# foges/pogs

Hardware: AMD Instinct MI355X
Metric: admm_iterations_per_sec_dense_lasso_fp32 (per-GPU shard, summed over GPUs) (higher is better)
Workload: dtype f32

## Files before the change

include/pogs_amd.h:

```cpp
#ifndef POGS_AMD_H_
#define POGS_AMD_H_

#include <stddef.h>

#ifdef __cplusplus
extern "C" {
#endif


enum ORD { COL_MAJ, ROW_MAJ };

enum FUNCTION { ABS, EXP, HUBER, IDENTITY, INDBOX01, INDEQ0, INDGE0, INDLE0,
                LOGISTIC, MAXNEG0, MAXPOS0, NEGENTR, NEGLOG, RECIPR, SQUARE, ZERO };

enum POGS_STATUS { POGS_SUCCESS = 0, POGS_INFEASIBLE = 1, POGS_UNBOUNDED = 2,
                   POGS_MAX_ITER = 3, POGS_NAN_FOUND = 4, POGS_INVALID_CONE = 5,
                   POGS_ERROR = 6 };

int PogsD(enum ORD ord, size_t m, size_t n, const double *A,
          const double *f_a, const double *f_b, const double *f_c,
          const double *f_d, const double *f_e, const enum FUNCTION *f_h,
          const double *g_a, const double *g_b, const double *g_c,
          const double *g_d, const double *g_e, const enum FUNCTION *g_h,
          double rho, double abs_tol, double rel_tol, unsigned int max_iter,
          unsigned int verbose, int adaptive_rho, int gap_stop,
          double *x, double *y, double *l, double *optval, unsigned int *final_iter);

int PogsS(enum ORD ord, size_t m, size_t n, const float *A,
          const float *f_a, const float *f_b, const float *f_c,
          const float *f_d, const float *f_e, const enum FUNCTION *f_h,
          const float *g_a, const float *g_b, const float *g_c,
          const float *g_d, const float *g_e, const enum FUNCTION *g_h,
          float rho, float abs_tol, float rel_tol, unsigned int max_iter,
          unsigned int verbose, int adaptive_rho, int gap_stop,
          float *x, float *y, float *l, float *optval, unsigned int *final_iter);

int PogsSparseD(enum ORD ord, size_t m, size_t n, size_t nnz,
                const double *data, const int *ptr, const int *ind,
                const double *f_a, const double *f_b, const double *f_c,
                const double *f_d, const double *f_e, const enum FUNCTION *f_h,
                const double *g_a, const double *g_b, const double *g_c,
                const double *g_d, const double *g_e, const enum FUNCTION *g_h,
                double rho, double abs_tol, double rel_tol, unsigned int max_iter,
                unsigned int verbose, int adaptive_rho, int gap_stop,
                double *x, double *y, double *l, double *optval,
                unsigned int *final_iter);

int PogsSparseS(enum ORD ord, size_t m, size_t n, size_t nnz,
                const float *data, const int *ptr, const int *ind,
                const float *f_a, const float *f_b, const float *f_c,
                const float *f_d, const float *f_e, const enum FUNCTION *f_h,
                const float *g_a, const float *g_b, const float *g_c,
                const float *g_d, const float *g_e, const enum FUNCTION *g_h,
                float rho, float abs_tol, float rel_tol, unsigned int max_iter,
                unsigned int verbose, int adaptive_rho, int gap_stop,
                float *x, float *y, float *l, float *optval,
                unsigned int *final_iter);


typedef struct PogsAmdSolver PogsAmdSolver;

enum POGS_AMD_DTYPE { POGS_AMD_F32 = 0, POGS_AMD_F64 = 1 };
enum POGS_AMD_MEM { POGS_AMD_HOST = 0, POGS_AMD_DEVICE = 1 };
enum POGS_AMD_PROJECTOR { POGS_AMD_PROJ_DEFAULT = 0,
                          POGS_AMD_PROJ_DIRECT = 1, POGS_AMD_PROJ_CGLS = 2 };

#define POGS_AMD_UNIQUE_ID_BYTES 128

typedef struct PogsAmdDist {
  int rank;
  int world;
  size_t m_global;
  char unique_id[POGS_AMD_UNIQUE_ID_BYTES];
} PogsAmdDist;

typedef struct PogsAmdOptions {
  int device;
  int projector;
  int profile;
  int reserved[5];
} PogsAmdOptions;

typedef struct PogsAmdStats {
  double t_total_s, t_init_s, t_loop_s, t_h2d_s;
  unsigned int iterations;
  unsigned int exact_iters;
  unsigned int norm_est_iters;
  unsigned int rho_updates;
  unsigned long long cg_iters;
  unsigned long long matvecs;
  unsigned long long matvecs_init;
  double rho_final, nrmA;
  double stream_ms;
  unsigned long long stream_launches;
  double stream_bytes;
  double equil_ms, normest_ms, gram_ms, chol_ms, trtri_ms;
  double gram_flops;
  double reserved[8];
} PogsAmdStats;

int PogsAmdDistUniqueId(char *out);

int PogsAmdCreateDense(PogsAmdSolver **out, int dtype, enum ORD ord, size_t m,
                       size_t n, const void *A, int mem,
                       const PogsAmdOptions *opt, const PogsAmdDist *dist);

int PogsAmdCreateSparse(PogsAmdSolver **out, int dtype, enum ORD ord, size_t m,
                        size_t n, size_t nnz, const void *data, const int *ptr,
                        const int *ind, int mem, const PogsAmdOptions *opt,
                        const PogsAmdDist *dist);

int PogsAmdSolve(PogsAmdSolver *s,
                 const void *f_a, const void *f_b, const void *f_c, const void *f_d,
                 const void *f_e, const int *f_h,
                 const void *g_a, const void *g_b, const void *g_c, const void *g_d,
                 const void *g_e, const int *g_h,
                 double rho, double abs_tol, double rel_tol, unsigned int max_iter,
                 unsigned int verbose, int adaptive_rho, int gap_stop,
                 void *x, void *y, void *l, void *mu, double *optval,
                 unsigned int *final_iter);

typedef struct PogsAmdFn {
  const void *a, *b, *c, *d, *e;
  const int *h;
  double a0, b0, c0, d0, e0;
  int h0;
} PogsAmdFn;
int PogsAmdSolveFn(PogsAmdSolver *s, const PogsAmdFn *f, const PogsAmdFn *g,
                   double rho, double abs_tol, double rel_tol, unsigned int max_iter,
                   unsigned int verbose, int adaptive_rho, int gap_stop,
                   void *x, void *y, void *l, void *mu, double *optval,
                   unsigned int *final_iter);
int PogsAmdBeginRunFn(PogsAmdSolver *s, const PogsAmdFn *f, const PogsAmdFn *g,
                      double rho, double abs_tol, double rel_tol, unsigned int max_iter,
                      int adaptive_rho, int gap_stop);

#define POGS_AMD_BATCH_MAX 16
int PogsAmdSolveBatchFn(PogsAmdSolver *s, int k, const PogsAmdFn *f, const PogsAmdFn *g, const double *rho,
                        double abs_tol, double rel_tol, unsigned int max_iter, unsigned int verbose,
                        int adaptive_rho, int gap_stop, void *x, void *y, void *l, void *mu,
                        double *optval, unsigned int *final_iter, int *status);

int PogsAmdSolveBatchSparseFn(PogsAmdSolver *s, int k, const PogsAmdFn *f, const PogsAmdFn *g, const double *rho,
                              double abs_tol, double rel_tol, unsigned int max_iter, unsigned int verbose,
                              int adaptive_rho, int gap_stop, void *x, void *y, void *l, void *mu,
                              double *optval, unsigned int *final_iter, int *status);

#define POGS_AMD_MANY_MIN_DIM_MAX 512
#define POGS_AMD_MANY_MAX_DIM_MAX 16384
int PogsAmdSolveManyFn(int dtype, enum ORD ord, int k, size_t m, size_t n, const void *A, int mem,
                       const PogsAmdOptions *opt, const PogsAmdFn *f, const PogsAmdFn *g, const double *rho,
                       double abs_tol, double rel_tol, unsigned int max_iter, unsigned int verbose,
                       int adaptive_rho, int gap_stop, void *x, void *y, void *l, void *mu,
                       double *optval, unsigned int *final_iter, int *status);

int PogsAmdBeginRun(PogsAmdSolver *s,
                    const void *f_a, const void *f_b, const void *f_c, const void *f_d,
                    const void *f_e, const int *f_h,
                    const void *g_a, const void *g_b, const void *g_c, const void *g_d,
                    const void *g_e, const int *g_h,
                    double rho, double abs_tol, double rel_tol, unsigned int max_iter,
                    int adaptive_rho, int gap_stop);
int PogsAmdIterate(PogsAmdSolver *s, unsigned int iters, double *seconds,
                   unsigned int *solves_completed);

int PogsAmdSetWarmStart(PogsAmdSolver *s, const void *x0, const void *l0);

int PogsAmdGetStats(const PogsAmdSolver *s, PogsAmdStats *out);
int PogsAmdResetStats(PogsAmdSolver *s);
void PogsAmdDestroy(PogsAmdSolver *s);

const char *PogsAmdLastError(void);

typedef struct PogsAmdPoolInfo {
  unsigned long long mallocs;
  unsigned long long reuses;
  unsigned long long frees;
  double malloc_ms, free_ms;
  size_t cached_bytes;
  size_t live_bytes;
  size_t peak_cached_bytes;
} PogsAmdPoolInfo;
int PogsAmdPoolStats(int device, PogsAmdPoolInfo *out);
int PogsAmdPoolTrim(int device, size_t *freed_bytes);


int PogsAmdProxEval(int dtype, size_t n, const int *h, const void *a, const void *b,
                    const void *c, const void *d, const void *e, double rho,
                    const void *in, void *out);
int PogsAmdFuncEval(int dtype, size_t n, const int *h, const void *a, const void *b,
                    const void *c, const void *d, const void *e, const void *in,
                    double *out);
int PogsAmdProjSubgradEval(int dtype, size_t n, const int *h, const void *a, const void *b,
                           const void *c, const void *d, const void *e, const void *x_in,
                           const void *v_in, void *v_out);
int PogsAmdGetEquil(const PogsAmdSolver *s, void *A_eq, void *d, void *e, double *nrmA);
int PogsAmdProject(PogsAmdSolver *s, const void *x0, const void *y0, double tol,
                   void *x, void *y);
int PogsAmdMul(PogsAmdSolver *s, char trans, double alpha, const void *x, double beta,
               void *y);
int PogsAmdReadBandwidth(int device, size_t bytes, int reps, double *gb_per_s, int *pattern);
int PogsAmdWaveSumCheck(int dtype, size_t n, const void *in_host, void *alu_host, void *lds_host);

int PogsAmdBatchRowsCheck(int dtype, int tri, int rows, int cols, const void *M, size_t ldm, int k, const int *act,
                          int nact, const void *X, size_t ldx, void *Y, size_t ldy);
int PogsAmdBatchColsCheck(int dtype, int rows, int cols, const void *M, size_t ldm, int k, const int *act, int nact,
                          const void *U, size_t ldu, const void *add, void *Z, size_t ldz, int *nrb_used, int *rpb);
int PogsAmdSpBatchSpmvCheck(int dtype, int nrows, int ncols, const int *ptr, const int *ind, const void *val, int k,
                            const int *act, int nact, const void *X, size_t ldx, double beta, const void *yin,
                            size_t ldin, void *Y, size_t ldy, double *part, int num_cu, int *geom);
int PogsAmdManySetupCheck(int dtype, enum ORD ord, int k, size_t m, size_t n, const void *A, int mem, void *A_eq,
                          void *d, void *e, double *nrmA, void *W);
int PogsAmdGramCheck(int dtype, int kdim, int k, const void *P, size_t lda, int num_cu, int force, void *G, size_t ldg,
                     int *info);
int PogsAmdCholCheck(int dtype, int n, const void *H, size_t ldh, void *L, void *W, void *U, size_t ldo);
int PogsAmdSpmvCheck(int dtype, enum ORD ord, int nrows, int ncols, const int *ptr, const int *ind, const void *val,
                     int num_cu, int format, int force_rr_rows, int force_ncg, double scale, char trans, int sq,
                     double x_nrm2, double alpha, double beta, const void *x, size_t xlen, void *y, size_t ylen,
                     double *sumsq, int *info, int *t_ptr, int *t_ind, void *t_val);
int PogsAmdGetFactor(const PogsAmdSolver *s, void *W, void *U);
int PogsAmdRandUniform(int dtype, size_t n, void *out_host);

#ifdef __cplusplus
}
#endif
#endif
```

pogs_amd/_lib.py:

```python
import ctypes
import os
import sys

_PKG = os.path.dirname(os.path.abspath(__file__))
LIB_PATH = os.path.join(_PKG, "libpogs_amd.so")

TORCH_LOADED_FIRST = "torch" in sys.modules
if not TORCH_LOADED_FIRST and os.environ.get("POGS_AMD_TORCH_PRELOAD", "0") == "1":
    try:
        import torch

        TORCH_LOADED_FIRST = True
    except ImportError:
        pass


def check_device_pointer_interop():
    if "torch" in sys.modules and not TORCH_LOADED_FIRST:
        raise RuntimeError(
            "pogs_amd was imported before torch: the two then run on separate HIP runtimes and a torch device "
            "pointer is not valid here.  Import torch first, or set POGS_AMD_TORCH_PRELOAD=1.")


if not os.path.exists(LIB_PATH):
    raise ImportError(
        "pogs_amd: %s not found. Build it with:\n"
        "  python pogs_amd/build.py        (needs hipcc; cross-compiles for gfx950 without a GPU)\n" % LIB_PATH
    )

lib = ctypes.CDLL(LIB_PATH)

c_int, c_uint, c_size_t, c_double, c_float, c_void_p, c_char = (
    ctypes.c_int, ctypes.c_uint, ctypes.c_size_t, ctypes.c_double, ctypes.c_float, ctypes.c_void_p, ctypes.c_char)

UNIQUE_ID_BYTES = 128
F32, F64 = 0, 1
HOST, DEVICE = 0, 1
COL_MAJ, ROW_MAJ = 0, 1
PROJ_DEFAULT, PROJ_DIRECT, PROJ_CGLS = 0, 1, 2


class PogsAmdDist(ctypes.Structure):
    _fields_ = [("rank", c_int), ("world", c_int), ("m_global", c_size_t), ("unique_id", c_char * UNIQUE_ID_BYTES)]


class PogsAmdOptions(ctypes.Structure):
    _fields_ = [("device", c_int), ("projector", c_int), ("profile", c_int), ("reserved", c_int * 5)]


class PogsAmdStats(ctypes.Structure):
    _fields_ = [
        ("t_total_s", c_double), ("t_init_s", c_double), ("t_loop_s", c_double), ("t_h2d_s", c_double),
        ("iterations", c_uint), ("exact_iters", c_uint), ("norm_est_iters", c_uint), ("rho_updates", c_uint),
        ("cg_iters", ctypes.c_ulonglong), ("matvecs", ctypes.c_ulonglong), ("matvecs_init", ctypes.c_ulonglong),
        ("rho_final", c_double), ("nrmA", c_double),
        ("stream_ms", c_double), ("stream_launches", ctypes.c_ulonglong), ("stream_bytes", c_double),
        ("equil_ms", c_double), ("normest_ms", c_double), ("gram_ms", c_double), ("chol_ms", c_double),
        ("trtri_ms", c_double), ("gram_flops", c_double), ("reserved", c_double * 8),
    ]

    def as_dict(self):
        d = {k: getattr(self, k) for k, _ in self._fields_ if k != "reserved"}
        d["spec_hits"], d["spec_misses"] = self.reserved[0], self.reserved[1]
        d["collectives"] = int(self.reserved[2])
        d["comm_nranks"] = int(self.reserved[3])
        d["batch_problem_iters"] = int(self.reserved[4])
        d["batch_pass_ms"], d["batch_pass_launches"] = self.reserved[5], int(self.reserved[6])
        d["batch_pass_bytes"] = self.reserved[7]
        return d


def _dense_sig(real):
    return [c_int, c_size_t, c_size_t, c_void_p] + [c_void_p] * 5 + [c_void_p] + [c_void_p] * 5 + [c_void_p] + \
        [real, real, real, c_uint, c_uint, c_int, c_int, c_void_p, c_void_p, c_void_p, c_void_p, c_void_p]


def _sparse_sig(real):
    return [c_int, c_size_t, c_size_t, c_size_t, c_void_p, c_void_p, c_void_p] + [c_void_p] * 5 + [c_void_p] + \
        [c_void_p] * 5 + [c_void_p] + [real, real, real, c_uint, c_uint, c_int, c_int,
                                        c_void_p, c_void_p, c_void_p, c_void_p, c_void_p]


lib.PogsD.argtypes = _dense_sig(c_double)
lib.PogsS.argtypes = _dense_sig(c_float)
lib.PogsSparseD.argtypes = _sparse_sig(c_double)
lib.PogsSparseS.argtypes = _sparse_sig(c_float)
for _f in (lib.PogsD, lib.PogsS, lib.PogsSparseD, lib.PogsSparseS):
    _f.restype = c_int

lib.PogsAmdDistUniqueId.argtypes = [c_void_p]
lib.PogsAmdCreateDense.argtypes = [ctypes.POINTER(c_void_p), c_int, c_int, c_size_t, c_size_t, c_void_p, c_int,
                                   ctypes.POINTER(PogsAmdOptions), ctypes.POINTER(PogsAmdDist)]
lib.PogsAmdCreateSparse.argtypes = [ctypes.POINTER(c_void_p), c_int, c_int, c_size_t, c_size_t, c_size_t, c_void_p,
                                    c_void_p, c_void_p, c_int, ctypes.POINTER(PogsAmdOptions),
                                    ctypes.POINTER(PogsAmdDist)]
lib.PogsAmdSolve.argtypes = [c_void_p] + [c_void_p] * 12 + [c_double, c_double, c_double, c_uint, c_uint, c_int, c_int,
                                                            c_void_p, c_void_p, c_void_p, c_void_p,
                                                            ctypes.POINTER(c_double), ctypes.POINTER(c_uint)]
class PogsAmdFn(ctypes.Structure):
    _fields_ = [("a", c_void_p), ("b", c_void_p), ("c", c_void_p), ("d", c_void_p), ("e", c_void_p), ("h", c_void_p),
                ("a0", c_double), ("b0", c_double), ("c0", c_double), ("d0", c_double), ("e0", c_double), ("h0", c_int)]


lib.PogsAmdSolveFn.argtypes = [c_void_p, ctypes.POINTER(PogsAmdFn), ctypes.POINTER(PogsAmdFn), c_double, c_double, c_double,
                               c_uint, c_uint, c_int, c_int, c_void_p, c_void_p, c_void_p, c_void_p,
                               ctypes.POINTER(c_double), ctypes.POINTER(c_uint)]
lib.PogsAmdSolveBatchFn.argtypes = [c_void_p, c_int, ctypes.POINTER(PogsAmdFn), ctypes.POINTER(PogsAmdFn), c_void_p,
                                    c_double, c_double, c_uint, c_uint, c_int, c_int, c_void_p, c_void_p, c_void_p,
                                    c_void_p, c_void_p, c_void_p, c_void_p]
lib.PogsAmdSolveBatchSparseFn.argtypes = lib.PogsAmdSolveBatchFn.argtypes
BATCH_MAX = 16
lib.PogsAmdSolveManyFn.argtypes = [c_int, c_int, c_int, c_size_t, c_size_t, c_void_p, c_int, ctypes.POINTER(PogsAmdOptions),
                                   ctypes.POINTER(PogsAmdFn), ctypes.POINTER(PogsAmdFn), c_void_p, c_double, c_double,
                                   c_uint, c_uint, c_int, c_int, c_void_p, c_void_p, c_void_p, c_void_p, c_void_p,
                                   c_void_p, c_void_p]
MANY_MIN_DIM_MAX = 512
MANY_MAX_DIM_MAX = 16384
lib.PogsAmdBeginRunFn.argtypes = [c_void_p, ctypes.POINTER(PogsAmdFn), ctypes.POINTER(PogsAmdFn), c_double, c_double, c_double,
                                  c_uint, c_int, c_int]
lib.PogsAmdBeginRun.argtypes = [c_void_p] + [c_void_p] * 12 + [c_double, c_double, c_double, c_uint, c_int, c_int]
lib.PogsAmdIterate.argtypes = [c_void_p, c_uint, ctypes.POINTER(c_double), ctypes.POINTER(c_uint)]
lib.PogsAmdSetWarmStart.argtypes = [c_void_p, c_void_p, c_void_p]
lib.PogsAmdGetStats.argtypes = [c_void_p, ctypes.POINTER(PogsAmdStats)]
lib.PogsAmdResetStats.argtypes = [c_void_p]
lib.PogsAmdDestroy.argtypes = [c_void_p]
lib.PogsAmdDestroy.restype = None
lib.PogsAmdLastError.restype = ctypes.c_char_p
lib.PogsAmdProxEval.argtypes = [c_int, c_size_t] + [c_void_p] * 6 + [c_double, c_void_p, c_void_p]
lib.PogsAmdFuncEval.argtypes = [c_int, c_size_t] + [c_void_p] * 6 + [c_void_p, ctypes.POINTER(c_double)]
lib.PogsAmdProjSubgradEval.argtypes = [c_int, c_size_t] + [c_void_p] * 6 + [c_void_p, c_void_p, c_void_p]
lib.PogsAmdGetEquil.argtypes = [c_void_p, c_void_p, c_void_p, c_void_p, ctypes.POINTER(c_double)]
lib.PogsAmdProject.argtypes = [c_void_p, c_void_p, c_void_p, c_double, c_void_p, c_void_p]
lib.PogsAmdMul.argtypes = [c_void_p, c_char, c_double, c_void_p, c_double, c_void_p]
lib.PogsAmdRandUniform.argtypes = [c_int, c_size_t, c_void_p]
lib.PogsAmdReadBandwidth.argtypes = [c_int, c_size_t, c_int, ctypes.POINTER(c_double), ctypes.POINTER(c_int)]
lib.PogsAmdWaveSumCheck.argtypes = [c_int, c_size_t, c_void_p, c_void_p, c_void_p]
lib.PogsAmdBatchRowsCheck.argtypes = [c_int, c_int, c_int, c_int, c_void_p, c_size_t, c_int, c_void_p, c_int,
                                      c_void_p, c_size_t, c_void_p, c_size_t]
lib.PogsAmdBatchColsCheck.argtypes = [c_int, c_int, c_int, c_void_p, c_size_t, c_int, c_void_p, c_int, c_void_p,
                                      c_size_t, c_void_p, c_void_p, c_size_t, ctypes.POINTER(c_int),
                                      ctypes.POINTER(c_int)]
lib.PogsAmdSpBatchSpmvCheck.argtypes = [c_int, c_int, c_int, c_void_p, c_void_p, c_void_p, c_int, c_void_p, c_int,
                                        c_void_p, c_size_t, c_double, c_void_p, c_size_t, c_void_p, c_size_t, c_void_p,
                                        c_int, c_void_p]
lib.PogsAmdManySetupCheck.argtypes = [c_int, c_int, c_int, c_size_t, c_size_t, c_void_p, c_int, c_void_p, c_void_p,
                                      c_void_p, c_void_p, c_void_p]
lib.PogsAmdGramCheck.argtypes = [c_int, c_int, c_int, c_void_p, c_size_t, c_int, c_int, c_void_p, c_size_t, c_void_p]
lib.PogsAmdCholCheck.argtypes = [c_int, c_int, c_void_p, c_size_t, c_void_p, c_void_p, c_void_p, c_size_t]
lib.PogsAmdSpmvCheck.argtypes = [c_int, c_int, c_int, c_int, c_void_p, c_void_p, c_void_p, c_int, c_int, c_int, c_int,
                                 c_double, c_char, c_int, c_double, c_double, c_double, c_void_p, c_size_t, c_void_p,
                                 c_size_t, ctypes.POINTER(c_double), c_void_p, c_void_p, c_void_p, c_void_p]
lib.PogsAmdGetFactor.argtypes = [c_void_p, c_void_p, c_void_p]
GRAM_AUTO, GRAM_NATIVE, GRAM_TILE_128, GRAM_TILE_256 = 0, 1, 128, 256
GRAM_INFO = ("path", "tile", "ksplit", "kchunk", "kacc", "units", "unit_rows", "tile_map")
SPMV_AUTO, SPMV_TAGS, SPMV_TWO, SPMV_PLAIN = 0, 1, 2, 3
SPMV_INFO = ("tiled", "two", "rr_rows", "nrr", "ncb", "ncg", "units", "why")
SPMV_WHY = {0: "tiled", 1: "no non-zeros", 2: "plan too large", 3: "planner range", 4: "padding", 5: "row count over 16 bits",
            6: "pinned plain"}


class PogsAmdPoolInfo(ctypes.Structure):
    _fields_ = [("mallocs", ctypes.c_ulonglong), ("reuses", ctypes.c_ulonglong), ("frees", ctypes.c_ulonglong),
                ("malloc_ms", c_double), ("free_ms", c_double), ("cached_bytes", c_size_t), ("live_bytes", c_size_t),
                ("peak_cached_bytes", c_size_t)]


lib.PogsAmdPoolStats.argtypes = [c_int, ctypes.POINTER(PogsAmdPoolInfo)]
lib.PogsAmdPoolTrim.argtypes = [c_int, ctypes.POINTER(c_size_t)]


def pool_stats(device=-1):
    info = PogsAmdPoolInfo()
    if lib.PogsAmdPoolStats(device, ctypes.byref(info)) != 0:
        raise RuntimeError(last_error())
    return {k: getattr(info, k) for k, _ in info._fields_}


def pool_trim(device=-1):
    freed = c_size_t(0)
    if lib.PogsAmdPoolTrim(device, ctypes.byref(freed)) != 0:
        raise RuntimeError(last_error())
    return freed.value

ABI_SYMBOLS = [
    "PogsD", "PogsS", "PogsSparseD", "PogsSparseS",
    "PogsAmdDistUniqueId", "PogsAmdCreateDense", "PogsAmdCreateSparse", "PogsAmdSolve", "PogsAmdSolveFn", "PogsAmdSolveBatchFn", "PogsAmdSolveBatchSparseFn",
    "PogsAmdSolveManyFn", "PogsAmdBeginRun", "PogsAmdBeginRunFn",
    "PogsAmdIterate", "PogsAmdSetWarmStart", "PogsAmdGetStats", "PogsAmdResetStats", "PogsAmdDestroy", "PogsAmdLastError",
    "PogsAmdPoolStats", "PogsAmdPoolTrim",
    "PogsAmdProxEval", "PogsAmdFuncEval", "PogsAmdProjSubgradEval", "PogsAmdGetEquil", "PogsAmdProject", "PogsAmdMul", "PogsAmdRandUniform",
    "PogsAmdReadBandwidth", "PogsAmdWaveSumCheck", "PogsAmdBatchRowsCheck", "PogsAmdBatchColsCheck",
    "PogsAmdSpBatchSpmvCheck", "PogsAmdManySetupCheck", "PogsAmdGramCheck", "PogsAmdCholCheck",
    "PogsAmdSpmvCheck", "PogsAmdGetFactor",
]


def read_bandwidth(device=-1, nbytes=4 << 30, reps=10):
    gbs, pat = c_double(0.0), c_int(0)
    if lib.PogsAmdReadBandwidth(device, nbytes, reps, ctypes.byref(gbs), ctypes.byref(pat)) != 0:
        raise RuntimeError(last_error())
    return gbs.value, ("side-by-side grid stride", "row blocks")[pat.value]


def wave_sum_check(values):
    import numpy as np
    v = np.ascontiguousarray(values)
    assert v.dtype in (np.float32, np.float64) and v.size % 64 == 0
    a, b = np.empty_like(v), np.empty_like(v)
    if lib.PogsAmdWaveSumCheck(0 if v.dtype == np.float32 else 1, v.size, v.ctypes.data, a.ctypes.data, b.ctypes.data) != 0:
        raise RuntimeError(last_error())
    return a, b


def _dtype_code(*arrays):
    import numpy as np
    dt = arrays[0].dtype
    if dt not in (np.float32, np.float64) or any(a.dtype != dt for a in arrays[1:]):
        raise ValueError("float32 or float64 arrays of one dtype")
    return 0 if dt == np.float32 else 1


def _act(act):
    import numpy as np
    return np.ascontiguousarray(act, dtype=np.int32).ravel()


def batch_rows_check(tri, M, cols, X, Y, act):
    import numpy as np
    M, X = np.ascontiguousarray(M), np.ascontiguousarray(X)
    Y = np.array(Y, order="C", copy=True)
    code = _dtype_code(M, X, Y)
    if M.ndim != 2 or X.ndim != 2 or Y.ndim != 2 or X.shape[0] != Y.shape[0]:
        raise ValueError("M (rows, ldm), X (k, ldx), Y (k, ldy)")
    a = _act(act)
    if lib.PogsAmdBatchRowsCheck(code, tri, M.shape[0], cols, M.ctypes.data, M.shape[1], X.shape[0], a.ctypes.data,
                                 a.size, X.ctypes.data, X.shape[1], Y.ctypes.data, Y.shape[1]) != 0:
        raise RuntimeError(last_error())
    return Y


def batch_cols_check(M, cols, U, Z, act, add=None):
    import numpy as np
    M, U = np.ascontiguousarray(M), np.ascontiguousarray(U)
    Z = np.array(Z, order="C", copy=True)
    arrays = (M, U, Z) if add is None else (M, U, Z, np.ascontiguousarray(add))
    code = _dtype_code(*arrays)
    if M.ndim != 2 or U.ndim != 2 or Z.ndim != 2 or U.shape[0] != Z.shape[0] or \
            (add is not None and arrays[3].shape != Z.shape):
        raise ValueError("M (rows, ldm), U (k, ldu), Z and add (k, ldz)")
    a = _act(act)
    nrb, rpb = c_int(0), c_int(0)
    if lib.PogsAmdBatchColsCheck(code, M.shape[0], cols, M.ctypes.data, M.shape[1], U.shape[0], a.ctypes.data, a.size,
                                 U.ctypes.data, U.shape[1], None if add is None else arrays[3].ctypes.data,
                                 Z.ctypes.data, Z.shape[1], ctypes.byref(nrb), ctypes.byref(rpb)) != 0:
        raise RuntimeError(last_error())
    return Z, nrb.value, rpb.value


def sp_batch_spmv_check(ptr, ind, val, ncols, X, Y, act, beta=0.0, yin=None, part_fill=None, num_cu=0):
    import numpy as np
    ptr, ind = np.ascontiguousarray(ptr, dtype=np.int32), np.ascontiguousarray(ind, dtype=np.int32)
    val, X = np.ascontiguousarray(val), np.ascontiguousarray(X)
    Y = np.array(Y, order="C", copy=True)
    arrays = (val, X, Y) if yin is None else (val, X, Y, np.ascontiguousarray(yin))
    code = _dtype_code(*arrays)
    nrows = ptr.size - 1
    if X.ndim != 2 or Y.ndim != 2 or X.shape[0] != Y.shape[0] or nrows < 0 or \
            (yin is not None and (arrays[3].ndim != 2 or arrays[3].shape[0] != Y.shape[0])):
        raise ValueError("ptr (nrows + 1), X (k, ldx), Y (k, ldy), yin (k, ldin)")
    nnz = max(int(ptr[-1]), 0) if ptr.size else 0
    if ind.size < nnz or val.size < nnz:
        raise ValueError("ind and val must hold ptr[-1] entries")
    a = _act(act)
    k = X.shape[0]
    part = None
    if part_fill is not None:
        part = np.full(k * max(1, -(-nrows // 4)), part_fill, dtype=np.float64)
    geom = np.zeros(3, dtype=np.int32)
    if lib.PogsAmdSpBatchSpmvCheck(code, nrows, ncols, ptr.ctypes.data, ind.ctypes.data, val.ctypes.data, k,
                                   a.ctypes.data, a.size, X.ctypes.data, X.shape[1], beta,
                                   None if yin is None else arrays[3].ctypes.data,
                                   0 if yin is None else arrays[3].shape[1], Y.ctypes.data, Y.shape[1],
                                   None if part is None else part.ctypes.data, num_cu, geom.ctypes.data) != 0:
        raise RuntimeError(last_error())
    grid = int(geom[2])
    return Y, (None if part is None else part[:k * grid].reshape(k, grid)), tuple(int(g) for g in geom)


def many_setup_check(A, ord=ROW_MAJ):
    import numpy as np
    A = np.asarray(A)
    if A.ndim != 3:
        raise ValueError("A must be k x m x n")
    code = _dtype_code(A)
    k, m, n = A.shape
    src = np.ascontiguousarray(A.transpose(0, 2, 1) if ord == COL_MAJ else A)
    K = min(m, n)
    out = dict(A_eq=np.empty((k, m, n), A.dtype), d=np.empty((k, m), A.dtype), e=np.empty((k, n), A.dtype),
               nrmA=np.empty(k, np.float64), W=np.empty((k, K, K), A.dtype))
    if lib.PogsAmdManySetupCheck(code, ord, k, m, n, src.ctypes.data, HOST, out["A_eq"].ctypes.data,
                                 out["d"].ctypes.data, out["e"].ctypes.data, out["nrmA"].ctypes.data,
                                 out["W"].ctypes.data) != 0:
        raise RuntimeError(last_error())
    return out


def gram_check(P, k, G, force=GRAM_AUTO, num_cu=0):
    import numpy as np
    P = np.ascontiguousarray(P)
    G = np.array(G, order="C", copy=True)
    code = _dtype_code(P, G)
    if P.ndim != 2 or G.ndim != 2 or G.shape[0] != k:
        raise ValueError("P (kdim, lda), G (k, ldg)")
    info = np.zeros(8, dtype=np.int32)
    if lib.PogsAmdGramCheck(code, P.shape[0], k, P.ctypes.data, P.shape[1], num_cu, force, G.ctypes.data, G.shape[1],
                            info.ctypes.data) != 0:
        raise RuntimeError(last_error())
    return G, dict(zip(GRAM_INFO, (int(v) for v in info)))


def spmv_check(ptr, ind, val, shape, x, y, trans="n", ord=ROW_MAJ, num_cu=0, format=SPMV_AUTO, force_rr_rows=0,
               force_ncg=0, scale=1.0, sq=False, x_nrm2=0.0, alpha=1.0, beta=0.0, transpose=False):
    import numpy as np
    ptr, ind = np.ascontiguousarray(ptr, dtype=np.int32), np.ascontiguousarray(ind, dtype=np.int32)
    val, x = np.ascontiguousarray(val), np.ascontiguousarray(x)
    y = np.array(y, order="C", copy=True)
    code = _dtype_code(val, x, y)
    nrows, ncols = int(shape[0]), int(shape[1])
    r1, c1 = (nrows, ncols) if ord == ROW_MAJ else (ncols, nrows)
    if ptr.ndim != 1 or ptr.size != r1 + 1 or x.ndim != 1 or y.ndim != 1:
        raise ValueError("ptr (rows of the given copy + 1), x and y vectors")
    nnz = max(int(ptr[-1]), 0)
    if ind.size < nnz or val.size < nnz:
        raise ValueError("ind and val must hold ptr[-1] entries")
    info = np.zeros(16, dtype=np.int32)
    sumsq = c_double(0.0)
    t = None
    if transpose:
        t = (np.zeros(c1 + 1, np.int32), np.zeros(max(nnz, 1), np.int32), np.zeros(max(nnz, 1), val.dtype))
    if lib.PogsAmdSpmvCheck(code, ord, nrows, ncols, ptr.ctypes.data, ind.ctypes.data, val.ctypes.data, num_cu, format,
                            force_rr_rows, force_ncg, scale, trans.encode(), int(bool(sq)), x_nrm2, alpha, beta,
                            x.ctypes.data, x.size, y.ctypes.data, y.size, ctypes.byref(sumsq), info.ctypes.data,
                            *((None, None, None) if t is None else (a.ctypes.data for a in t))) != 0:
        raise RuntimeError(last_error())
    infos = tuple(dict(zip(SPMV_INFO, (int(v) for v in info[8 * c:8 * c + 8]))) for c in range(2))
    if t is None:
        return y, sumsq.value, infos
    return y, sumsq.value, infos, (t[0], t[1][:nnz], t[2][:nnz])


def chol_check(H, ldo=None):
    import numpy as np
    H = np.ascontiguousarray(H)
    code = _dtype_code(H)
    if H.ndim != 2 or H.shape[1] < H.shape[0]:
        raise ValueError("H (n, ldh >= n)")
    n = H.shape[0]
    ldo = n if ldo is None else ldo
    L, W, U = (np.full((n, ldo), np.nan, H.dtype) for _ in range(3))
    if lib.PogsAmdCholCheck(code, n, H.ctypes.data, H.shape[1], L.ctypes.data, W.ctypes.data, U.ctypes.data, ldo) != 0:
        raise RuntimeError(last_error())
    return L, W, U


def get_factor(handle, k, dtype):
    import numpy as np
    W, U = np.zeros((k, k), dtype), np.zeros((k, k), dtype)
    if lib.PogsAmdGetFactor(handle, W.ctypes.data, U.ctypes.data) != 0:
        raise RuntimeError(last_error())
    return W, U


def last_error():
    msg = lib.PogsAmdLastError()
    return msg.decode() if msg else ""
```

pogs_amd/csrc/abi.hip:

```cpp
#include <cmath>
#include <cstring>
#include <string>
#include <utility>
#include <vector>

#include "engine.h"
#include "factor_check.h"
#include "many_kernels.h"
#include "sparse_batch_kernels.h"
#include "spmv_check.h"
#include "prox.h"
#include "stream.h"
#include "vec_kernels.h"

namespace pogs_amd {

#define POGS_DECLARE_PLAN(TPB_, NV_)                                                                               \
  SolverBase *make_dense_solver_f32_p##TPB_##_##NV_(int, size_t, size_t, const void *, int, const PogsAmdOptions *, \
                                                    const PogsAmdDist *);                                          \
  SolverBase *make_dense_solver_f64_p##TPB_##_##NV_(int, size_t, size_t, const void *, int, const PogsAmdOptions *, \
                                                    const PogsAmdDist *);
POGS_STREAM_PLANS(POGS_DECLARE_PLAN)
#undef POGS_DECLARE_PLAN
SolverBase *make_dense_solver_f32_xl(int, size_t, size_t, const void *, int, const PogsAmdOptions *, const PogsAmdDist *);
SolverBase *make_dense_solver_f64_xl(int, size_t, size_t, const void *, int, const PogsAmdOptions *, const PogsAmdDist *);

template <typename T>
inline StreamPlan dense_plan_for(size_t m, size_t n, const PogsAmdOptions *opt, const PogsAmdDist *dist) {
  const size_t m_global = (dist && dist->world >= 1) ? dist->m_global : m;
  const bool tall = m_global > n;
  const bool cgls = opt && opt->projector == POGS_AMD_PROJ_CGLS;
  const size_t stored_cols = (!tall && !cgls) ? m : n;
  return make_stream_plan<T>(static_cast<int>(round_up(stored_cols, Vec16<T>::N)), 256);
}

inline SolverBase *make_dense_solver(int dtype, int ord, size_t m, size_t n, const void *A, int mem,
                                     const PogsAmdOptions *opt, const PogsAmdDist *dist) {
  POGS_CHECK(dtype == POGS_AMD_F32 || dtype == POGS_AMD_F64, "unknown dtype");
  POGS_CHECK(m > 0 && n > 0 && m < (1u << 31) && n < (1u << 31), "bad dimensions");
  const bool f32 = dtype == POGS_AMD_F32;
  const StreamPlan p = f32 ? dense_plan_for<float>(m, n, opt, dist) : dense_plan_for<double>(m, n, opt, dist);
  POGS_CHECK(p.ok, "no streaming shape for this matrix");
  if (p.xl) return f32 ? make_dense_solver_f32_xl(ord, m, n, A, mem, opt, dist) : make_dense_solver_f64_xl(ord, m, n, A, mem, opt, dist);
#define POGS_PICK_PLAN(TPB_, NV_)                                                          \
  if (p.tpb == TPB_ && p.nv == NV_)                                                        \
    return f32 ? make_dense_solver_f32_p##TPB_##_##NV_(ord, m, n, A, mem, opt, dist)       \
               : make_dense_solver_f64_p##TPB_##_##NV_(ord, m, n, A, mem, opt, dist);
  POGS_STREAM_PLANS(POGS_PICK_PLAN)
#undef POGS_PICK_PLAN
  throw Error("no dense solver for this streaming shape");
}
SolverBase *make_sparse_solver(int dtype, int ord, size_t m, size_t n, size_t nnz, const void *data,
                               const int *ptr, const int *ind, int mem, const PogsAmdOptions *opt,
                               const PogsAmdDist *dist);

namespace {
struct MinStd0 {
  uint64_t s = 1;
  uint32_t next() {
    s = (s * 16807ull) % 2147483647ull;
    return static_cast<uint32_t>(s);
  }
};
}
void rand_uniform_host(float *x, size_t n) {
  MinStd0 g;
  const float r = static_cast<float>(2147483646.0L);
  for (size_t i = 0; i < n; ++i) {
    float v = static_cast<float>(g.next() - 1u) / r;
    if (v >= 1.0f) v = std::nextafter(1.0f, 0.0f);
    x[i] = v;
  }
}
void rand_uniform_host(double *x, size_t n) {
  MinStd0 g;
  const double r = 2147483646.0;
  for (size_t i = 0; i < n; ++i) {
    const double lo = static_cast<double>(g.next() - 1u);
    const double hi = static_cast<double>(g.next() - 1u);
    double v = (lo + hi * r) / (r * r);
    if (v >= 1.0) v = std::nextafter(1.0, 0.0);
    x[i] = v;
  }
}

namespace {

thread_local std::string g_last_error;

template <typename F>
int guarded(F &&fn, PogsAmdSolver *h = nullptr) {
  auto failed = [&](const char *what) {
    g_last_error = what;
    std::fprintf(stderr, "pogs_amd: %s\n", what);
    try {
      if (h && h->impl) h->impl->on_error();
    } catch (...) {}
    return POGS_ERROR;
  };
  try {
    g_last_error.clear();
    if (h && h->impl) h->impl->on_entry();
    return fn();
  } catch (const std::exception &e) {
    return failed(e.what());
  } catch (...) {
    return failed("unknown error");
  }
}

SolveParams make_params(double rho, double abs_tol, double rel_tol, unsigned max_iter, unsigned verbose,
                        int adaptive_rho, int gap_stop) {
  SolveParams p;
  p.rho = rho; p.abs_tol = abs_tol; p.rel_tol = rel_tol;
  p.max_iter = max_iter == 0 ? 1 : max_iter;
  p.verbose = verbose;
  p.adaptive_rho = adaptive_rho != 0;
  p.gap_stop = gap_stop != 0;
  return p;
}

FnHost fn_arrays(const void *a, const void *b, const void *c, const void *d, const void *e, const int *h, const char *which) {
  if (!(a && b && c && d && e && h))
    throw Error(std::string("null coefficient array in the description of ") + which +
                " (a, b, c, d, e, h must all be given; broadcast fields: PogsAmdSolveFn)");
  return FnHost{a, b, c, d, e, h};
}

template <typename T>
int pogs_dense(enum ORD ord, size_t m, size_t n, const T *A, const T *f_a, const T *f_b, const T *f_c,
               const T *f_d, const T *f_e, const enum FUNCTION *f_h, const T *g_a, const T *g_b, const T *g_c,
               const T *g_d, const T *g_e, const enum FUNCTION *g_h, T rho, T abs_tol, T rel_tol,
               unsigned max_iter, unsigned verbose, int adaptive_rho, int gap_stop, T *x, T *y, T *l, T *optval,
               unsigned *final_iter) {
  return guarded([&]() {
    const FnHost f = fn_arrays(f_a, f_b, f_c, f_d, f_e, reinterpret_cast<const int *>(f_h), "f");
    const FnHost g = fn_arrays(g_a, g_b, g_c, g_d, g_e, reinterpret_cast<const int *>(g_h), "g");
    std::unique_ptr<SolverBase> s(make_dense_solver(sizeof(T) == 4 ? POGS_AMD_F32 : POGS_AMD_F64, ord, m, n, A,
                                                    POGS_AMD_HOST, nullptr, nullptr));
    double ov = 0;
    const int st = s->solve(f, g, make_params(rho, abs_tol, rel_tol, max_iter, verbose, adaptive_rho, gap_stop),
                            x, y, l, nullptr, &ov, final_iter);
    *optval = static_cast<T>(ov);
    return st;
  });
}

template <typename T>
int pogs_sparse(enum ORD ord, size_t m, size_t n, size_t nnz, const T *data, const int *ptr, const int *ind,
                const T *f_a, const T *f_b, const T *f_c, const T *f_d, const T *f_e, const enum FUNCTION *f_h,
                const T *g_a, const T *g_b, const T *g_c, const T *g_d, const T *g_e, const enum FUNCTION *g_h,
                T rho, T abs_tol, T rel_tol, unsigned max_iter, unsigned verbose, int adaptive_rho, int gap_stop,
                T *x, T *y, T *l, T *optval, unsigned *final_iter) {
  return guarded([&]() {
    const FnHost f = fn_arrays(f_a, f_b, f_c, f_d, f_e, reinterpret_cast<const int *>(f_h), "f");
    const FnHost g = fn_arrays(g_a, g_b, g_c, g_d, g_e, reinterpret_cast<const int *>(g_h), "g");
    std::unique_ptr<SolverBase> s(make_sparse_solver(sizeof(T) == 4 ? POGS_AMD_F32 : POGS_AMD_F64, ord, m, n, nnz,
                                                     data, ptr, ind, POGS_AMD_HOST, nullptr, nullptr));
    double ov = 0;
    const int st = s->solve(f, g, make_params(rho, abs_tol, rel_tol, max_iter, verbose, adaptive_rho, gap_stop),
                            x, y, l, nullptr, &ov, final_iter);
    *optval = static_cast<T>(ov);
    return st;
  });
}

template <typename T>
void prox_eval_host(size_t n, const int *h, const void *a, const void *b, const void *c, const void *d,
                    const void *e, double rho, const void *in, void *out, double *fsum, const void *xin = nullptr) {
  POGS_CHECK(n < (1u << 31), "n too large");
  hipStream_t s = nullptr;
  const int cnt = static_cast<int>(n);
  FnBuf<T> fb;
  fb.alloc(n);
  DevBuf<T> vin(n), vout(n);
  auto up = [&](void *dst, const void *src, size_t bytes) {
    POGS_HIP_CHECK(hipMemcpyAsync(dst, src, bytes, hipMemcpyHostToDevice, s));
  };
  up(fb.h.p, h, n * sizeof(int));
  up(fb.a.p, a, n * sizeof(T)); up(fb.b.p, b, n * sizeof(T)); up(fb.c.p, c, n * sizeof(T));
  up(fb.d.p, d, n * sizeof(T)); up(fb.e.p, e, n * sizeof(T));
  up(vin.p, in, n * sizeof(T));
  {
    FnHost fh{a, b, c, d, e, h};
    warn_negative_coeffs<T>(fh, n);
  }
  DevBuf<T> ones(n);
  launch_fill<T>(ones.p, static_cast<T>(1), n, s);
  launch_scale_objective<T>(fb.view(), fb.a.p, fb.c.p, fb.d.p, fb.e.p, ones.p, cnt, false, s);
  if (out && xin) {
    DevBuf<T> xv(n);
    up(xv.p, xin, n * sizeof(T));
    launch_proj_subgrad<T>(cnt, fb.view(), xv.p, vin.p, vout.p, s);
    POGS_HIP_CHECK(hipMemcpyAsync(out, vout.p, n * sizeof(T), hipMemcpyDeviceToHost, s));
    POGS_HIP_CHECK(hipStreamSynchronize(s));
  } else if (out) {
    launch_prox_eval<T>(cnt, fb.view(), static_cast<T>(rho), vin.p, vout.p, s);
    POGS_HIP_CHECK(hipMemcpyAsync(out, vout.p, n * sizeof(T), hipMemcpyDeviceToHost, s));
  }
  if (fsum) {
    const int blocks = vec_blocks(cnt);
    DevBuf<double> part(blocks), tot(1);
    launch_func_eval<T>(cnt, fb.view(), vin.p, part.p, s);
    SumJob j{part.p, blocks, 1, tot.p};
    launch_sum_jobs(&j, 1, s);
    POGS_HIP_CHECK(hipMemcpyAsync(fsum, tot.p, sizeof(double), hipMemcpyDeviceToHost, s));
    POGS_HIP_CHECK(hipStreamSynchronize(s));
  }
  POGS_HIP_CHECK(hipStreamSynchronize(s));
}

}
}

using namespace pogs_amd;

extern "C" {

int PogsD(enum ORD ord, size_t m, size_t n, const double *A, const double *f_a, const double *f_b,
          const double *f_c, const double *f_d, const double *f_e, const enum FUNCTION *f_h, const double *g_a,
          const double *g_b, const double *g_c, const double *g_d, const double *g_e, const enum FUNCTION *g_h,
          double rho, double abs_tol, double rel_tol, unsigned int max_iter, unsigned int verbose,
          int adaptive_rho, int gap_stop, double *x, double *y, double *l, double *optval,
          unsigned int *final_iter) {
  return pogs_dense<double>(ord, m, n, A, f_a, f_b, f_c, f_d, f_e, f_h, g_a, g_b, g_c, g_d, g_e, g_h, rho, abs_tol,
                            rel_tol, max_iter, verbose, adaptive_rho, gap_stop, x, y, l, optval, final_iter);
}

int PogsS(enum ORD ord, size_t m, size_t n, const float *A, const float *f_a, const float *f_b, const float *f_c,
          const float *f_d, const float *f_e, const enum FUNCTION *f_h, const float *g_a, const float *g_b,
          const float *g_c, const float *g_d, const float *g_e, const enum FUNCTION *g_h, float rho, float abs_tol,
          float rel_tol, unsigned int max_iter, unsigned int verbose, int adaptive_rho, int gap_stop, float *x,
          float *y, float *l, float *optval, unsigned int *final_iter) {
  return pogs_dense<float>(ord, m, n, A, f_a, f_b, f_c, f_d, f_e, f_h, g_a, g_b, g_c, g_d, g_e, g_h, rho, abs_tol,
                           rel_tol, max_iter, verbose, adaptive_rho, gap_stop, x, y, l, optval, final_iter);
}

int PogsSparseD(enum ORD ord, size_t m, size_t n, size_t nnz, const double *data, const int *ptr, const int *ind,
                const double *f_a, const double *f_b, const double *f_c, const double *f_d, const double *f_e,
                const enum FUNCTION *f_h, const double *g_a, const double *g_b, const double *g_c,
                const double *g_d, const double *g_e, const enum FUNCTION *g_h, double rho, double abs_tol,
                double rel_tol, unsigned int max_iter, unsigned int verbose, int adaptive_rho, int gap_stop,
                double *x, double *y, double *l, double *optval, unsigned int *final_iter) {
  return pogs_sparse<double>(ord, m, n, nnz, data, ptr, ind, f_a, f_b, f_c, f_d, f_e, f_h, g_a, g_b, g_c, g_d, g_e,
                             g_h, rho, abs_tol, rel_tol, max_iter, verbose, adaptive_rho, gap_stop, x, y, l, optval,
                             final_iter);
}

int PogsSparseS(enum ORD ord, size_t m, size_t n, size_t nnz, const float *data, const int *ptr, const int *ind,
                const float *f_a, const float *f_b, const float *f_c, const float *f_d, const float *f_e,
                const enum FUNCTION *f_h, const float *g_a, const float *g_b, const float *g_c, const float *g_d,
                const float *g_e, const enum FUNCTION *g_h, float rho, float abs_tol, float rel_tol,
                unsigned int max_iter, unsigned int verbose, int adaptive_rho, int gap_stop, float *x, float *y,
                float *l, float *optval, unsigned int *final_iter) {
  return pogs_sparse<float>(ord, m, n, nnz, data, ptr, ind, f_a, f_b, f_c, f_d, f_e, f_h, g_a, g_b, g_c, g_d, g_e,
                            g_h, rho, abs_tol, rel_tol, max_iter, verbose, adaptive_rho, gap_stop, x, y, l, optval,
                            final_iter);
}

int PogsAmdDistUniqueId(char *out) {
  return guarded([&]() {
    DistComm::unique_id(out);
    return 0;
  });
}

int PogsAmdCreateDense(PogsAmdSolver **out, int dtype, enum ORD ord, size_t m, size_t n, const void *A, int mem,
                       const PogsAmdOptions *opt, const PogsAmdDist *dist) {
  return guarded([&]() {
    *out = nullptr;
    DeviceGuard guard(opt ? opt->device : -1);
    std::unique_ptr<PogsAmdSolver> h(new PogsAmdSolver);
    h->impl.reset(make_dense_solver(dtype, ord, m, n, A, mem, opt, dist));
    *out = h.release();
    return 0;
  });
}

int PogsAmdCreateSparse(PogsAmdSolver **out, int dtype, enum ORD ord, size_t m, size_t n, size_t nnz,
                        const void *data, const int *ptr, const int *ind, int mem, const PogsAmdOptions *opt,
                        const PogsAmdDist *dist) {
  return guarded([&]() {
    *out = nullptr;
    DeviceGuard guard(opt ? opt->device : -1);
    std::unique_ptr<PogsAmdSolver> h(new PogsAmdSolver);
    h->impl.reset(make_sparse_solver(dtype, ord, m, n, nnz, data, ptr, ind, mem, opt, dist));
    *out = h.release();
    return 0;
  });
}

int PogsAmdSolve(PogsAmdSolver *s, const void *f_a, const void *f_b, const void *f_c, const void *f_d,
                 const void *f_e, const int *f_h, const void *g_a, const void *g_b, const void *g_c,
                 const void *g_d, const void *g_e, const int *g_h, double rho, double abs_tol, double rel_tol,
                 unsigned int max_iter, unsigned int verbose, int adaptive_rho, int gap_stop, void *x, void *y,
                 void *l, void *mu, double *optval, unsigned int *final_iter) {
  return guarded([&]() {
    POGS_CHECK(s && s->impl, "null solver");
    DeviceGuard guard(s->impl->device());
    const FnHost f = fn_arrays(f_a, f_b, f_c, f_d, f_e, f_h, "f");
    const FnHost g = fn_arrays(g_a, g_b, g_c, g_d, g_e, g_h, "g");
    return s->impl->solve(f, g, make_params(rho, abs_tol, rel_tol, max_iter, verbose, adaptive_rho, gap_stop), x,
                          y, l, mu, optval, final_iter);
  }, s);
}

namespace {
FnHost fn_host(const PogsAmdFn *p) {
  POGS_CHECK(p != nullptr, "null function description");
  FnHost f{p->a, p->b, p->c, p->d, p->e, p->h};
  f.s0[0] = p->a0; f.s0[1] = p->b0; f.s0[2] = p->c0; f.s0[3] = p->d0; f.s0[4] = p->e0;
  f.h0 = p->h0;
  POGS_CHECK(p->h || (p->h0 >= 0 && p->h0 <= 15), "function code out of range");
  return f;
}
std::pair<std::vector<FnHost>, std::vector<FnHost>> fn_hosts(const std::string &what, int k, const PogsAmdFn *f,
                                                             const PogsAmdFn *g, const void *x,
                                                             const unsigned *final_iter, const int *status) {
  POGS_CHECK(f && g, (what + ": null function descriptions").c_str());
  POGS_CHECK(x && final_iter && status, (what + ": x, final_iter and status must not be NULL").c_str());
  std::pair<std::vector<FnHost>, std::vector<FnHost>> fg;
  for (int j = 0; j < k; ++j) {
    fg.first.push_back(fn_host(&f[j]));
    fg.second.push_back(fn_host(&g[j]));
  }
  return fg;
}
}

int PogsAmdSolveFn(PogsAmdSolver *s, const PogsAmdFn *f, const PogsAmdFn *g, double rho, double abs_tol, double rel_tol,
                   unsigned int max_iter, unsigned int verbose, int adaptive_rho, int gap_stop, void *x, void *y, void *l,
                   void *mu, double *optval, unsigned int *final_iter) {
  return guarded([&]() {
    POGS_CHECK(s && s->impl, "null solver");
    DeviceGuard guard(s->impl->device());
    const FnHost fh = fn_host(f), gh = fn_host(g);
    return s->impl->solve(fh, gh, make_params(rho, abs_tol, rel_tol, max_iter, verbose, adaptive_rho, gap_stop), x, y, l, mu,
                          optval, final_iter);
  }, s);
}

int PogsAmdSolveBatchFn(PogsAmdSolver *s, int k, const PogsAmdFn *f, const PogsAmdFn *g, const double *rho,
                        double abs_tol, double rel_tol, unsigned int max_iter, unsigned int verbose, int adaptive_rho,
                        int gap_stop, void *x, void *y, void *l, void *mu, double *optval, unsigned int *final_iter,
                        int *status) {
  return guarded([&]() {
    POGS_CHECK(s && s->impl, "null solver");
    POGS_CHECK(k >= 1 && k <= POGS_AMD_BATCH_MAX, "batched solve: k must be in [1, POGS_AMD_BATCH_MAX]");
    const auto fg = fn_hosts("batched solve", k, f, g, x, final_iter, status);
    DeviceGuard guard(s->impl->device());
    s->impl->solve_batch(k, fg.first.data(), fg.second.data(), rho,
                         make_params(1.0, abs_tol, rel_tol, max_iter, verbose, adaptive_rho, gap_stop),
                         BatchOut{x, y, l, mu, optval, final_iter, status});
    return 0;
  }, s);
}

int PogsAmdSolveBatchSparseFn(PogsAmdSolver *s, int k, const PogsAmdFn *f, const PogsAmdFn *g, const double *rho,
                              double abs_tol, double rel_tol, unsigned int max_iter, unsigned int verbose,
                              int adaptive_rho, int gap_stop, void *x, void *y, void *l, void *mu, double *optval,
                              unsigned int *final_iter, int *status) {
  return guarded([&]() {
    POGS_CHECK(s && s->impl, "null solver");
    POGS_CHECK(k >= 1 && k <= POGS_AMD_BATCH_MAX, "batched solve: k must be in [1, POGS_AMD_BATCH_MAX]");
    const auto fg = fn_hosts("batched solve", k, f, g, x, final_iter, status);
    DeviceGuard guard(s->impl->device());
    s->impl->solve_batch_sparse(k, fg.first.data(), fg.second.data(), rho,
                                make_params(1.0, abs_tol, rel_tol, max_iter, verbose, adaptive_rho, gap_stop),
                                BatchOut{x, y, l, mu, optval, final_iter, status});
    return 0;
  }, s);
}

int PogsAmdSolveManyFn(int dtype, enum ORD ord, int k, size_t m, size_t n, const void *A, int mem,
                       const PogsAmdOptions *opt, const PogsAmdFn *f, const PogsAmdFn *g, const double *rho,
                       double abs_tol, double rel_tol, unsigned int max_iter, unsigned int verbose, int adaptive_rho,
                       int gap_stop, void *x, void *y, void *l, void *mu, double *optval, unsigned int *final_iter,
                       int *status) {
  return guarded([&]() {
    POGS_CHECK(k >= 1, "many-problem solve: k must be >= 1");
    const int projector = opt ? opt->projector : POGS_AMD_PROJ_DEFAULT;
    POGS_CHECK(projector == POGS_AMD_PROJ_DEFAULT || projector == POGS_AMD_PROJ_DIRECT,
               "many-problem solve: only the direct projector is supported (CGLS refused)");
    const int device = opt ? opt->device : -1;
    const auto fg = fn_hosts("many-problem solve", k, f, g, x, final_iter, status);
    DeviceGuard guard(device);
    solve_many(dtype, static_cast<int>(ord), k, m, n, A, mem, device, fg.first.data(), fg.second.data(), rho,
               make_params(1.0, abs_tol, rel_tol, max_iter, verbose, adaptive_rho, gap_stop),
               BatchOut{x, y, l, mu, optval, final_iter, status});
    return 0;
  });
}

int PogsAmdBeginRunFn(PogsAmdSolver *s, const PogsAmdFn *f, const PogsAmdFn *g, double rho, double abs_tol, double rel_tol,
                      unsigned int max_iter, int adaptive_rho, int gap_stop) {
  return guarded([&]() {
    POGS_CHECK(s && s->impl, "null solver");
    DeviceGuard guard(s->impl->device());
    const FnHost fh = fn_host(f), gh = fn_host(g);
    s->impl->begin_run(fh, gh, make_params(rho, abs_tol, rel_tol, max_iter, 0, adaptive_rho, gap_stop));
    return 0;
  }, s);
}

int PogsAmdBeginRun(PogsAmdSolver *s, const void *f_a, const void *f_b, const void *f_c, const void *f_d,
                    const void *f_e, const int *f_h, const void *g_a, const void *g_b, const void *g_c,
                    const void *g_d, const void *g_e, const int *g_h, double rho, double abs_tol, double rel_tol,
                    unsigned int max_iter, int adaptive_rho, int gap_stop) {
  return guarded([&]() {
    POGS_CHECK(s && s->impl, "null solver");
    DeviceGuard guard(s->impl->device());
    const FnHost f = fn_arrays(f_a, f_b, f_c, f_d, f_e, f_h, "f");
    const FnHost g = fn_arrays(g_a, g_b, g_c, g_d, g_e, g_h, "g");
    s->impl->begin_run(f, g, make_params(rho, abs_tol, rel_tol, max_iter, 0, adaptive_rho, gap_stop));
    return 0;
  }, s);
}

int PogsAmdIterate(PogsAmdSolver *s, unsigned int iters, double *seconds, unsigned int *solves_completed) {
  return guarded([&]() {
    POGS_CHECK(s && s->impl, "null solver");
    DeviceGuard guard(s->impl->device());
    s->impl->iterate(iters, seconds, solves_completed);
    return 0;
  }, s);
}

int PogsAmdSetWarmStart(PogsAmdSolver *s, const void *x0, const void *l0) {
  return guarded([&]() {
    POGS_CHECK(s && s->impl && x0 && l0, "warm start needs both x0 and l0 (pogs.cpp:159-179)");
    DeviceGuard guard(s->impl->device());
    s->impl->set_warm_start(x0, l0);
    return 0;
  });
}

int PogsAmdGetStats(const PogsAmdSolver *s, PogsAmdStats *out) {
  return guarded([&]() {
    POGS_CHECK(s && s->impl && out, "null argument");
    *out = const_cast<PogsAmdSolver *>(s)->impl->stats();
    return 0;
  });
}

int PogsAmdResetStats(PogsAmdSolver *s) {
  return guarded([&]() {
    POGS_CHECK(s && s->impl, "null solver");
    DeviceGuard guard(s->impl->device());
    PogsAmdStats &st = s->impl->stats();
    st.t_loop_s = 0; st.iterations = 0; st.exact_iters = 0; st.rho_updates = 0;
    st.cg_iters = 0; st.matvecs = 0;
    st.stream_ms = 0; st.stream_launches = 0; st.stream_bytes = 0;
    st.reserved[0] = 0; st.reserved[1] = 0;
    return 0;
  });
}

void PogsAmdDestroy(PogsAmdSolver *s) {
  try {
    if (!s) return;
    DeviceGuard guard(s->impl ? s->impl->device() : -1);
    delete s;
  } catch (...) {}
}

const char *PogsAmdLastError(void) { return g_last_error.c_str(); }

int PogsAmdPoolStats(int device, PogsAmdPoolInfo *out) {
  return guarded([&]() {
    POGS_CHECK(out, "null argument");
    int dev = device;
    if (dev < 0) POGS_HIP_CHECK(hipGetDevice(&dev));
    const PoolCounters c = DevicePool::get().counters(dev);
    out->mallocs = c.mallocs; out->reuses = c.reuses; out->frees = c.frees;
    out->malloc_ms = c.malloc_ms; out->free_ms = c.free_ms;
    out->cached_bytes = c.cached_bytes; out->live_bytes = c.live_bytes;
    out->peak_cached_bytes = c.peak_cached_bytes;
    return 0;
  });
}

int PogsAmdPoolTrim(int device, size_t *freed_bytes) {
  return guarded([&]() {
    const size_t b = DevicePool::get().trim(device);
    if (freed_bytes) *freed_bytes = b;
    return 0;
  });
}

int PogsAmdProxEval(int dtype, size_t n, const int *h, const void *a, const void *b, const void *c, const void *d,
                    const void *e, double rho, const void *in, void *out) {
  return guarded([&]() {
    if (dtype == POGS_AMD_F32) prox_eval_host<float>(n, h, a, b, c, d, e, rho, in, out, nullptr);
    else prox_eval_host<double>(n, h, a, b, c, d, e, rho, in, out, nullptr);
    return 0;
  });
}

int PogsAmdFuncEval(int dtype, size_t n, const int *h, const void *a, const void *b, const void *c, const void *d,
                    const void *e, const void *in, double *out) {
  return guarded([&]() {
    if (dtype == POGS_AMD_F32) prox_eval_host<float>(n, h, a, b, c, d, e, 1.0, in, nullptr, out);
    else prox_eval_host<double>(n, h, a, b, c, d, e, 1.0, in, nullptr, out);
    return 0;
  });
}

int PogsAmdProjSubgradEval(int dtype, size_t n, const int *h, const void *a, const void *b, const void *c,
                           const void *d, const void *e, const void *x_in, const void *v_in, void *v_out) {
  return guarded([&]() {
    POGS_CHECK(x_in && v_in && v_out, "null argument");
    if (dtype == POGS_AMD_F32) prox_eval_host<float>(n, h, a, b, c, d, e, 1.0, v_in, v_out, nullptr, x_in);
    else prox_eval_host<double>(n, h, a, b, c, d, e, 1.0, v_in, v_out, nullptr, x_in);
    return 0;
  });
}

int PogsAmdGetEquil(const PogsAmdSolver *s, void *A_eq, void *d, void *e, double *nrmA) {
  return guarded([&]() {
    POGS_CHECK(s && s->impl, "null solver");
    DeviceGuard guard(s->impl->device());
    const_cast<PogsAmdSolver *>(s)->impl->get_equil(A_eq, d, e, nrmA);
    return 0;
  });
}

int PogsAmdProject(PogsAmdSolver *s, const void *x0, const void *y0, double tol, void *x, void *y) {
  return guarded([&]() {
    POGS_CHECK(s && s->impl, "null solver");
    DeviceGuard guard(s->impl->device());
    s->impl->project(x0, y0, tol, x, y);
    return 0;
  });
}

int PogsAmdMul(PogsAmdSolver *s, char trans, double alpha, const void *x, double beta, void *y) {
  return guarded([&]() {
    POGS_CHECK(s && s->impl, "null solver");
    DeviceGuard guard(s->impl->device());
    s->impl->mul(trans, alpha, x, beta, y);
    return 0;
  });
}

int PogsAmdReadBandwidth(int device, size_t bytes, int reps, double *gb_per_s, int *pattern) {
  return guarded([&]() {
    POGS_CHECK(gb_per_s && bytes >= (1u << 20), "null argument / fewer than 1 MiB");
    DeviceGuard guard(device);
    int pat = 0;
    *gb_per_s = measure_read_bandwidth_gbs(bytes, reps, &pat);
    if (pattern) *pattern = pat;
    return 0;
  });
}

int PogsAmdWaveSumCheck(int dtype, size_t n, const void *in_host, void *alu_host, void *lds_host) {
  return guarded([&]() {
    POGS_CHECK(in_host && alu_host && lds_host, "null argument");
    if (dtype == POGS_AMD_F32) wave_sum_check(static_cast<const float *>(in_host), n, static_cast<float *>(alu_host), static_cast<float *>(lds_host));
    else wave_sum_check(static_cast<const double *>(in_host), n, static_cast<double *>(alu_host), static_cast<double *>(lds_host));
    return 0;
  });
}

int PogsAmdBatchRowsCheck(int dtype, int tri, int rows, int cols, const void *M, size_t ldm, int k, const int *act,
                          int nact, const void *X, size_t ldx, void *Y, size_t ldy) {
  return guarded([&]() {
    POGS_CHECK(dtype == POGS_AMD_F32 || dtype == POGS_AMD_F64, "unknown dtype");
    if (dtype == POGS_AMD_F32)
      batch_rows_check<float>(tri, rows, cols, static_cast<const float *>(M), ldm, k, act, nact,
                              static_cast<const float *>(X), ldx, static_cast<float *>(Y), ldy);
    else
      batch_rows_check<double>(tri, rows, cols, static_cast<const double *>(M), ldm, k, act, nact,
                               static_cast<const double *>(X), ldx, static_cast<double *>(Y), ldy);
    return 0;
  });
}

int PogsAmdBatchColsCheck(int dtype, int rows, int cols, const void *M, size_t ldm, int k, const int *act, int nact,
                          const void *U, size_t ldu, const void *add, void *Z, size_t ldz, int *nrb_used, int *rpb) {
  return guarded([&]() {
    POGS_CHECK(dtype == POGS_AMD_F32 || dtype == POGS_AMD_F64, "unknown dtype");
    if (dtype == POGS_AMD_F32)
      batch_cols_check<float>(rows, cols, static_cast<const float *>(M), ldm, k, act, nact,
                              static_cast<const float *>(U), ldu, static_cast<const float *>(add),
                              static_cast<float *>(Z), ldz, nrb_used, rpb);
    else
      batch_cols_check<double>(rows, cols, static_cast<const double *>(M), ldm, k, act, nact,
                               static_cast<const double *>(U), ldu, static_cast<const double *>(add),
                               static_cast<double *>(Z), ldz, nrb_used, rpb);
    return 0;
  });
}

int PogsAmdSpBatchSpmvCheck(int dtype, int nrows, int ncols, const int *ptr, const int *ind, const void *val, int k,
                            const int *act, int nact, const void *X, size_t ldx, double beta, const void *yin,
                            size_t ldin, void *Y, size_t ldy, double *part, int num_cu, int *geom) {
  return guarded([&]() {
    POGS_CHECK(dtype == POGS_AMD_F32 || dtype == POGS_AMD_F64, "unknown dtype");
    if (dtype == POGS_AMD_F32)
      sp_batch_spmv_check<float>(nrows, ncols, ptr, ind, static_cast<const float *>(val), k, act, nact,
                                 static_cast<const float *>(X), ldx, static_cast<float>(beta),
                                 static_cast<const float *>(yin), ldin, static_cast<float *>(Y), ldy, part, num_cu,
                                 geom);
    else
      sp_batch_spmv_check<double>(nrows, ncols, ptr, ind, static_cast<const double *>(val), k, act, nact,
                                  static_cast<const double *>(X), ldx, beta, static_cast<const double *>(yin), ldin,
                                  static_cast<double *>(Y), ldy, part, num_cu, geom);
    return 0;
  });
}

int PogsAmdManySetupCheck(int dtype, enum ORD ord, int k, size_t m, size_t n, const void *A, int mem, void *A_eq,
                          void *d, void *e, double *nrmA, void *W) {
  return guarded([&]() {
    many_setup_check(dtype, static_cast<int>(ord), k, m, n, A, mem, A_eq, d, e, nrmA, W);
    return 0;
  });
}

int PogsAmdGramCheck(int dtype, int kdim, int k, const void *P, size_t lda, int num_cu, int force, void *G, size_t ldg,
                     int *info) {
  return guarded([&]() {
    POGS_CHECK(dtype == POGS_AMD_F32 || dtype == POGS_AMD_F64, "unknown dtype");
    if (dtype == POGS_AMD_F32)
      gram_check<float>(kdim, k, static_cast<const float *>(P), lda, num_cu, force, static_cast<float *>(G), ldg, info);
    else
      gram_check<double>(kdim, k, static_cast<const double *>(P), lda, num_cu, force, static_cast<double *>(G), ldg, info);
    return 0;
  });
}

int PogsAmdCholCheck(int dtype, int n, const void *H, size_t ldh, void *L, void *W, void *U, size_t ldo) {
  return guarded([&]() {
    POGS_CHECK(dtype == POGS_AMD_F32 || dtype == POGS_AMD_F64, "unknown dtype");
    if (dtype == POGS_AMD_F32)
      chol_check<float>(n, static_cast<const float *>(H), ldh, static_cast<float *>(L), static_cast<float *>(W),
                        static_cast<float *>(U), ldo);
    else
      chol_check<double>(n, static_cast<const double *>(H), ldh, static_cast<double *>(L), static_cast<double *>(W),
                         static_cast<double *>(U), ldo);
    return 0;
  });
}

int PogsAmdSpmvCheck(int dtype, enum ORD ord, int nrows, int ncols, const int *ptr, const int *ind, const void *val,
                     int num_cu, int format, int force_rr_rows, int force_ncg, double scale, char trans, int sq,
                     double x_nrm2, double alpha, double beta, const void *x, size_t xlen, void *y, size_t ylen,
                     double *sumsq, int *info, int *t_ptr, int *t_ind, void *t_val) {
  return guarded([&]() {
    const SpmvCheckArgs a{dtype, static_cast<int>(ord), nrows, ncols, ptr, ind, val, num_cu, format, force_rr_rows,
                          force_ncg, scale, trans, sq, x_nrm2, alpha, beta, x, xlen, y, ylen, sumsq, info, t_ptr, t_ind,
                          t_val};
    spmv_check(a);
    return 0;
  });
}

int PogsAmdGetFactor(const PogsAmdSolver *s, void *W, void *U) {
  return guarded([&]() {
    POGS_CHECK(s && s->impl, "null solver");
    DeviceGuard guard(s->impl->device());
    const_cast<PogsAmdSolver *>(s)->impl->get_factor(W, U);
    return 0;
  });
}

int PogsAmdRandUniform(int dtype, size_t n, void *out_host) {
  return guarded([&]() {
    if (dtype == POGS_AMD_F32) rand_uniform_host(static_cast<float *>(out_host), n);
    else rand_uniform_host(static_cast<double *>(out_host), n);
    return 0;
  });
}

}
```

pogs_amd/csrc/dense_plan.hip:

```cpp
#include "dense_solver.h"

#define POGS_CAT2(a, b) a##b
#define POGS_CAT(a, b) POGS_CAT2(a, b)

namespace pogs_amd {
#if defined(POGS_PLAN_XL)
using PlanTag = WindowPlans;
#else
using PlanTag = OnePlan<POGS_PLAN_TPB, POGS_PLAN_NV>;
#endif
SolverBase *POGS_CAT(make_dense_solver_, POGS_PLAN_NAME)(int ord, size_t m, size_t n, const void *A, int mem,
                                                          const PogsAmdOptions *opt, const PogsAmdDist *dist) {
  return make_dense_solver_t<POGS_PLAN_T, PlanTag>(ord, m, n, A, mem, opt, dist);
}
}
```

pogs_amd/csrc/fused_cols.h:

```cpp
#pragma once
#include <hip/hip_runtime.h>

#include "common.h"
#include "prox.h"
#include "reduce.h"
#include "stream.h"
#include "vec_kernels.h"

namespace pogs_amd {

template <typename T>
__device__ __forceinline__ typename Vec16<T>::type colsum_group(const T *partials, int nparts, int n_pad, int col, int g) {
  using V = typename Vec16<T>::type;
  V sum = dev::vzero<V>();
  int b = g;
  for (; b + 56 < nparts; b += 64) {
    V v[8];
#pragma unroll
    for (int q = 0; q < 8; ++q) v[q] = *reinterpret_cast<const V *>(partials + static_cast<size_t>(b + 8 * q) * n_pad + col);
#pragma unroll
    for (int q = 0; q < 8; ++q) dev::vadd(sum, v[q]);
  }
  for (; b < nparts; b += 8) {
    const V v = *reinterpret_cast<const V *>(partials + static_cast<size_t>(b) * n_pad + col);
    dev::vadd(sum, v);
  }
  return sum;
}

template <typename T>
struct PreColsArgs {
  const T *part0, *part1;
  int nparts;
  const double *tot64;
  int n, n_pad;
  FnView<T> g;
  const T *x_cur, *xt;
  T zt_scale, rho, alpha;
  T *x12, *xtemp;
  T *rhs;
  double *partials;
};

constexpr int kPreColsVecs = 16, kPreColsGroups = 16;
inline int pre_cols_grid(int n_pad, int vec) { return (n_pad / vec + kPreColsVecs - 1) / kPreColsVecs; }

template <typename T, bool SRC64>
__global__ void __launch_bounds__(256) pre_cols_kernel(PreColsArgs<T> a) {
  using V = typename Vec16<T>::type;
  constexpr int VEC = Vec16<T>::N;
  constexpr int NC = kPreColsVecs * VEC;
  __shared__ T s_v[2][kPreColsGroups][NC];
  __shared__ double s_red[4 * 4];
  const int cx = threadIdx.x % kPreColsVecs, g = threadIdx.x / kPreColsVecs;
  const int col0 = blockIdx.x * NC;
  if (!SRC64) {
    const int col = col0 + cx * VEC;
    V s0 = dev::vzero<V>(), s1 = dev::vzero<V>();
    if (col < a.n_pad) {
      V t0 = dev::vzero<V>(), t1 = dev::vzero<V>();
      int b = g;
      if (a.part1) {
        for (; b + kPreColsGroups < a.nparts; b += 2 * kPreColsGroups) {
          const V u0 = *reinterpret_cast<const V *>(a.part0 + static_cast<size_t>(b) * a.n_pad + col);
          const V u1 = *reinterpret_cast<const V *>(a.part1 + static_cast<size_t>(b) * a.n_pad + col);
          const V w0 = *reinterpret_cast<const V *>(a.part0 + static_cast<size_t>(b + kPreColsGroups) * a.n_pad + col);
          const V w1 = *reinterpret_cast<const V *>(a.part1 + static_cast<size_t>(b + kPreColsGroups) * a.n_pad + col);
          dev::vadd(s0, u0);
          dev::vadd(s1, u1);
          dev::vadd(t0, w0);
          dev::vadd(t1, w1);
        }
        if (b < a.nparts) {
          dev::vadd(s0, *reinterpret_cast<const V *>(a.part0 + static_cast<size_t>(b) * a.n_pad + col));
          dev::vadd(s1, *reinterpret_cast<const V *>(a.part1 + static_cast<size_t>(b) * a.n_pad + col));
        }
      } else {
        for (; b + kPreColsGroups < a.nparts; b += 2 * kPreColsGroups) {
          const V u0 = *reinterpret_cast<const V *>(a.part0 + static_cast<size_t>(b) * a.n_pad + col);
          const V w0 = *reinterpret_cast<const V *>(a.part0 + static_cast<size_t>(b + kPreColsGroups) * a.n_pad + col);
          dev::vadd(s0, u0);
          dev::vadd(t0, w0);
        }
        if (b < a.nparts)
          dev::vadd(s0, *reinterpret_cast<const V *>(a.part0 + static_cast<size_t>(b) * a.n_pad + col));
      }
      dev::vadd(s0, t0);
      dev::vadd(s1, t1);
    }
    *reinterpret_cast<V *>(&s_v[0][g][cx * VEC]) = s0;
    *reinterpret_cast<V *>(&s_v[1][g][cx * VEC]) = s1;
    __syncthreads();
  }
  double sacc[4] = {0.0, 0.0, 0.0, 0.0};
  const int j = col0 + static_cast<int>(threadIdx.x);
  if (threadIdx.x < NC && j < a.n_pad) {
    T t0, t1;
    if (SRC64) {
      t0 = static_cast<T>(a.tot64[j]);
      t1 = static_cast<T>(a.tot64[a.n_pad + j]);
    } else {
      t0 = s_v[0][0][threadIdx.x];
      t1 = s_v[1][0][threadIdx.x];
#pragma unroll
      for (int q = 1; q < kPreColsGroups; ++q) {
        t0 += s_v[0][q][threadIdx.x];
        t1 += s_v[1][q][threadIdx.x];
      }
    }
    if (j < a.n) {
      const T prev = a.x_cur[j];
      const T xtj = a.xt[j];
      const T ztv = a.zt_scale * xtj;
      const T v = prev - ztv;
      const T h = dev::ProxEval(a.g.h[j], a.g.a[j], a.g.b[j], a.g.c[j], a.g.d[j], a.g.e[j], v, a.rho);
      const T w = v - h;
      a.x12[j] = h;
      a.xtemp[j] = ztv + a.alpha * h + (static_cast<T>(1) - a.alpha) * prev;
      sacc[0] = static_cast<double>(w) * h;
      sacc[1] = static_cast<double>(w) * w;
      sacc[2] = static_cast<double>(h) * h;
      a.rhs[j] = t0;
      const T sd = t1 + h + a.zt_scale * xtj - prev;
      sacc[3] = (SRC64 || a.part1) ? static_cast<double>(sd) * sd : 0.0;
    } else {
      a.rhs[j] = static_cast<T>(0);
    }
  }
  __syncthreads();
  dev::block_sum<4, 256>(sacc, s_red);
  if (threadIdx.x == 0) {
#pragma unroll
    for (int k = 0; k < 4; ++k) a.partials[static_cast<size_t>(blockIdx.x) * 4 + k] = sacc[k];
  }
}

template <typename T>
void launch_pre_cols(const PreColsArgs<T> &a, bool src64, hipStream_t s) {
  const int grid = pre_cols_grid(a.n_pad, Vec16<T>::N);
  if (src64) hipLaunchKernelGGL((pre_cols_kernel<T, true>), dim3(grid), dim3(256), 0, s, a);
  else hipLaunchKernelGGL((pre_cols_kernel<T, false>), dim3(grid), dim3(256), 0, s, a);
}

struct PackJobs {
  SumJob j[2];
  int njobs;
};
template <typename T>
__global__ void __launch_bounds__(256) pack_cols_kernel(const T *part0, const T *part1, int nparts, int n_pad,
                                                        double *pack, PackJobs jobs) {
  using V = typename Vec16<T>::type;
  constexpr int VEC = Vec16<T>::N;
  __shared__ V s_v[2][8][32];
  __shared__ double s_w[4];
  const int ncb = (n_pad / VEC + 31) / 32;
  if (static_cast<int>(blockIdx.x) == ncb) {
    const int t = threadIdx.x, lane = t & 63, wave = t >> 6;
    double *out = pack + 2 * static_cast<size_t>(n_pad);
    for (int q = 0; q < jobs.njobs; ++q) {
      const SumJob job = jobs.j[q];
      const size_t stride = job.stride > 0 ? job.stride : job.ns;
      for (int k = 0; k < job.ns; ++k) {
        const double *p = job.partials + job.offset + k;
        double sum = 0;
        for (int b = t; b < job.nparts; b += 256) sum += p[static_cast<size_t>(b) * stride];
        sum = dev::wave_sum(sum);
        if (lane == 0) s_w[wave] = sum;
        __syncthreads();
        if (t == 0) *out = (s_w[0] + s_w[1]) + (s_w[2] + s_w[3]);
        ++out;
        __syncthreads();
      }
    }
    return;
  }
  const int cx = threadIdx.x & 31, g = threadIdx.x >> 5;
  const int col = (blockIdx.x * 32 + cx) * VEC;
  V s0 = dev::vzero<V>(), s1 = dev::vzero<V>();
  if (col < n_pad) {
    s0 = colsum_group<T>(part0, nparts, n_pad, col, g);
    s1 = colsum_group<T>(part1, nparts, n_pad, col, g);
  }
  s_v[0][g][cx] = s0;
  s_v[1][g][cx] = s1;
  __syncthreads();
  if (g == 0 && col < n_pad) {
    V tot0 = s_v[0][0][cx], tot1 = s_v[1][0][cx];
#pragma unroll
    for (int q = 1; q < 8; ++q) {
      dev::vadd(tot0, s_v[0][q][cx]);
      dev::vadd(tot1, s_v[1][q][cx]);
    }
    T t0[VEC], t1[VEC];
    __builtin_memcpy(t0, &tot0, sizeof(V));
    __builtin_memcpy(t1, &tot1, sizeof(V));
#pragma unroll
    for (int i = 0; i < VEC; ++i) {
      pack[col + i] = static_cast<double>(t0[i]);
      pack[n_pad + col + i] = static_cast<double>(t1[i]);
    }
  }
}

template <typename T>
void launch_pack_cols(const T *part0, const T *part1, int nparts, int n_pad, double *pack, const PackJobs &jobs,
                      hipStream_t s) {
  const int grid = reduce_cols_grid(n_pad, Vec16<T>::N) + 1;
  hipLaunchKernelGGL((pack_cols_kernel<T>), dim3(grid), dim3(256), 0, s, part0, part1, nparts, n_pad, pack, jobs);
}

}
```

pogs_amd/csrc/stream.h:

```cpp
#pragma once
#include <atomic>
#include <cstdlib>
#include <hip/hip_runtime.h>

#include "common.h"
#include "reduce.h"

namespace pogs_amd {

#ifndef POGS_AMD_NT_LOADS
#define POGS_AMD_NT_LOADS 1
#endif
template <typename V, typename T>
__device__ __forceinline__ V stream_load(const T *p) {
#if POGS_AMD_NT_LOADS
  typedef unsigned int raw16 __attribute__((ext_vector_type(4)));
  static_assert(sizeof(V) == 16, "16-byte vectors");
  const raw16 raw = __builtin_nontemporal_load(reinterpret_cast<const raw16 *>(p));
  V out;
  __builtin_memcpy(&out, &raw, 16);
  return out;
#else
  return *reinterpret_cast<const V *>(p);
#endif
}

enum Tri : int { kFull = 0, kLower = 1, kUpper = 2 };

template <typename T>
struct StreamArgs {
  const T *A;
  size_t lda;
  int m;
  int n_pad;
  const T *xin;
  const T *xin_add;
  const double *xin_nrm2;
  T *col_partials;
  double *scalar_partials;
  int col0 = 0;
  T *xl_scratch = nullptr;
};

struct StreamPlan {
  int tpb = 0;
  int nv = 0;
  int grid_max = 0;
  int grid_dot = 0;
  int num_cu = 0;
  bool ok = false;
  bool xl = false;
  int bpc_override = 0;
  bool pf = false;
};
template <typename T> inline int stream_window_cols(const StreamPlan &p) { return p.tpb * p.nv * Vec16<T>::N; }
template <typename T> inline int stream_windows(const StreamPlan &p, int n_pad) {
  const int w = stream_window_cols<T>(p);
  return p.xl ? (n_pad + w - 1) / w : 1;
}
template <typename T> inline size_t stream_xl_scratch(const StreamPlan &p, int rows, int n_pad) {
  return p.xl ? static_cast<size_t>(stream_windows<T>(p, n_pad) + 1) * rows : 0;
}

#define POGS_STREAM_PLANS(X) \
  X(64, 1) X(64, 2) X(64, 4) X(256, 2) X(256, 3) X(256, 4) X(256, 5) X(256, 6) X(256, 8) X(256, 10) \
  X(512, 6) X(512, 8) X(512, 10) X(1024, 6) X(1024, 8)
struct AllPlans {
  static constexpr bool has(int, int) { return true; }
  static constexpr bool windows = true;
};
template <int TPB, int NV>
struct OnePlan {
  static constexpr bool has(int t, int v) { return t == TPB && v == NV; }
  static constexpr bool windows = false;
};
struct WindowPlans {
  static constexpr bool has(int, int) { return false; }
  static constexpr bool windows = true;
};

#ifndef POGS_C3_LEAN_BLOCKS
#define POGS_C3_LEAN_BLOCKS 3
#endif
#ifndef POGS_C3_FULL_BLOCKS
#define POGS_C3_FULL_BLOCKS 3
#endif
constexpr int stream2_blocks_per_cu(int tpb, int nv, int nd = 2, int na = 2) {
  return tpb == 64 ? 8
         : tpb == 256 ? (nv == 5 ? ((nd == 1 && na == 1) ? POGS_C3_LEAN_BLOCKS : POGS_C3_FULL_BLOCKS) : nv <= 2 ? 3 : 2)
                      : 1;
}
constexpr int stream2_waves_per_simd(int tpb, int nv, int nd = 2, int na = 2) {
  return (stream2_blocks_per_cu(tpb, nv, nd, na) * (tpb / 64) + 3) / 4;
}

template <typename T>
inline StreamPlan make_stream_plan(int n_pad, int num_cu) {
  constexpr int VEC = Vec16<T>::N;
  const int vpr = n_pad / VEC;
  StreamPlan p;
  static const int nv64[] = {1, 2, 4};
  static const int nv256[] = {2, 3, 4, 5, 6, 8, 10};
  static const int nv512[] = {6, 8, 10};
  static const int nv1024[] = {6, 8};
  const char *xl_env = std::getenv("POGS_AMD_XL_LIMIT");
  const bool forced_xl = xl_env && vpr > std::atoi(xl_env);
  for (int nv : nv64)
    if (!forced_xl && vpr <= 64 * nv) { p.tpb = 64; p.nv = nv; p.grid_max = p.grid_dot = num_cu * 8; p.ok = true; return p; }
  for (int nv : nv256)
    if (!forced_xl && vpr <= 256 * nv) {
      p.tpb = 256; p.nv = nv; p.grid_dot = num_cu * 2;
      p.num_cu = num_cu;
      p.grid_max = num_cu * std::max(stream2_blocks_per_cu(256, nv), stream2_blocks_per_cu(256, nv, 1, 1));
      p.ok = true;
      return p;
    }
  for (int nv : nv512)
    if (!forced_xl && vpr <= 512 * nv) { p.tpb = 512; p.nv = nv; p.grid_max = p.grid_dot = num_cu; p.ok = true; return p; }
  int limit = 1024 * 8;
  bool small_windows = false;
  if (const char *ev = std::getenv("POGS_AMD_XL_LIMIT")) { limit = std::atoi(ev); small_windows = true; }
  if (vpr <= limit) {
    for (int nv : nv1024)
      if (vpr <= 1024 * nv) { p.tpb = 1024; p.nv = nv; p.grid_max = p.grid_dot = num_cu; p.ok = true; return p; }
  }
  p.xl = true;
  p.ok = true;
  if (small_windows) { p.tpb = 64; p.nv = 2; p.grid_max = p.grid_dot = num_cu * 8; }
  else { p.tpb = 256; p.nv = 8; p.grid_max = p.grid_dot = num_cu * 2; }
  return p;
}

namespace dev {

__device__ __forceinline__ float vdot(const float4 &a, const float4 &b) {
  return fma_(a.w, b.w, fma_(a.z, b.z, fma_(a.y, b.y, a.x * b.x)));
}
__device__ __forceinline__ double vdot(const double2 &a, const double2 &b) {
  return fma_(a.y, b.y, a.x * b.x);
}
__device__ __forceinline__ void vfma(float4 &acc, float u, const float4 &a) {
  acc.x = fma_(u, a.x, acc.x); acc.y = fma_(u, a.y, acc.y); acc.z = fma_(u, a.z, acc.z); acc.w = fma_(u, a.w, acc.w);
}
__device__ __forceinline__ void vfma(double2 &acc, double u, const double2 &a) {
  acc.x = fma_(u, a.x, acc.x); acc.y = fma_(u, a.y, acc.y);
}
__device__ __forceinline__ void vadd(float4 &acc, const float4 &a) {
  acc.x += a.x; acc.y += a.y; acc.z += a.z; acc.w += a.w;
}
__device__ __forceinline__ void vadd(double2 &acc, const double2 &a) {
  acc.x += a.x; acc.y += a.y;
}
__device__ __forceinline__ float4 vsq(const float4 &a) {
  return make_float4(a.x * a.x, a.y * a.y, a.z * a.z, a.w * a.w);
}
__device__ __forceinline__ double2 vsq(const double2 &a) { return make_double2(a.x * a.x, a.y * a.y); }
__device__ __forceinline__ float4 vscale_add(const float4 &a, float s, const float4 &b) {
  return make_float4(fma_(a.x, s, b.x), fma_(a.y, s, b.y), fma_(a.z, s, b.z), fma_(a.w, s, b.w));
}
__device__ __forceinline__ double2 vscale_add(const double2 &a, double s, const double2 &b) {
  return make_double2(fma_(a.x, s, b.x), fma_(a.y, s, b.y));
}
template <typename V> __device__ __forceinline__ V vzero();
template <> __device__ __forceinline__ float4 vzero<float4>() { return make_float4(0.f, 0.f, 0.f, 0.f); }
template <> __device__ __forceinline__ double2 vzero<double2>() { return make_double2(0.0, 0.0); }

}

template <typename T, int TPB, int NV, int R, bool DOT, bool ACC, bool SQ, int TRI, typename Op>
__global__ void __launch_bounds__(TPB) stream_rows_kernel(StreamArgs<T> a, Op op) {
  using V = typename Vec16<T>::type;
  constexpr int VEC = Vec16<T>::N;
  constexpr int NW = TPB / 64;
  constexpr int NS = Op::NS > 0 ? Op::NS : 1;
  __shared__ T s_part[2 * R * NW];
  __shared__ T s_u[2 * R];
  __shared__ double s_red[NS * NW];

  const int t = threadIdx.x, lane = t & 63, wave = t >> 6;

  V xv[NV];
  V acc[NV];
  if (DOT) {
    T sc = 1;
    if (a.xin_nrm2) sc = static_cast<T>(1.0 / sqrt(*a.xin_nrm2));
#pragma unroll
    for (int v = 0; v < NV; ++v) {
      const int col = a.col0 + (v * TPB + t) * VEC;
      V x = dev::vzero<V>();
      if (col < a.n_pad) {
        x = *reinterpret_cast<const V *>(a.xin + col);
        V add = dev::vzero<V>();
        if (a.xin_add) add = *reinterpret_cast<const V *>(a.xin_add + col);
        x = dev::vscale_add(x, sc, add);
      }
      xv[v] = x;
    }
  }
  if (ACC) {
#pragma unroll
    for (int v = 0; v < NV; ++v) acc[v] = dev::vzero<V>();
  }
  double sacc[NS];
#pragma unroll
  for (int k = 0; k < NS; ++k) sacc[k] = 0.0;

  const int nblk = (a.m + R - 1) / R;
  int slot = 0;
  for (int blk = blockIdx.x; blk < nblk; blk += gridDim.x, slot ^= 1) {
    const int row0 = blk * R;
    V av[R][NV];
#pragma unroll
    for (int r = 0; r < R; ++r) {
      const int row = row0 + r;
      const T *rp = a.A + static_cast<size_t>(row) * a.lda;
#pragma unroll
      for (int v = 0; v < NV; ++v) {
        const int col = a.col0 + (v * TPB + t) * VEC;
        bool ok = (col < a.n_pad) && (row < a.m);
        if (TRI == kLower) ok = ok && (col <= row);
        if (TRI == kUpper) ok = ok && (col + VEC - 1 >= row);
        V val = dev::vzero<V>();
        if (ok) val = (TRI == kFull) ? stream_load<V>(rp + col) : *reinterpret_cast<const V *>(rp + col);
        av[r][v] = SQ ? dev::vsq(val) : val;
      }
    }
    if (DOT) {
      T p[R];
#pragma unroll
      for (int r = 0; r < R; ++r) {
        T s = 0;
#pragma unroll
        for (int v = 0; v < NV; ++v) s += dev::vdot(av[r][v], xv[v]);
        p[r] = dev::wave_sum(s);
      }
      if (lane == 0) {
#pragma unroll
        for (int r = 0; r < R; ++r) s_part[(slot * R + r) * NW + wave] = p[r];
      }
      __syncthreads();
      if (t < R) {
        const int row = row0 + t;
        T uval = 0;
        if (row < a.m) {
          T dot = 0;
#pragma unroll
          for (int w = 0; w < NW; ++w) dot += s_part[(slot * R + t) * NW + w];
          uval = op.row(row, dot, sacc);
        }
        if (ACC) s_u[slot * R + t] = uval;
      }
      if (ACC) __syncthreads();
    }
    if (ACC) {
#pragma unroll
      for (int r = 0; r < R; ++r) {
        T u;
        if (DOT) {
          u = s_u[slot * R + r];
        } else {
          u = (row0 + r < a.m) ? op.u(row0 + r) : static_cast<T>(0);
        }
#pragma unroll
        for (int v = 0; v < NV; ++v) dev::vfma(acc[v], u, av[r][v]);
      }
    }
  }
  if (ACC) {
    T *out = a.col_partials + static_cast<size_t>(blockIdx.x) * a.n_pad;
#pragma unroll
    for (int v = 0; v < NV; ++v) {
      const int col = a.col0 + (v * TPB + t) * VEC;
      if (col < a.n_pad) *reinterpret_cast<V *>(out + col) = acc[v];
    }
  }
  if (Op::NS > 0) {
    __syncthreads();
    dev::block_sum<NS, TPB>(sacc, s_red);
    if (t == 0) {
#pragma unroll
      for (int k = 0; k < NS; ++k) a.scalar_partials[static_cast<size_t>(blockIdx.x) * NS + k] = sacc[k];
    }
  }
}

template <typename T, int TPB, int NV, int RP, int NVP, int RMAX, int NSX, typename Op>
__device__ __forceinline__ void stream_tri_phase(const StreamArgs<T> &a, const Op &op, int row_begin, int row_end,
                                                 int blk_base, const typename Vec16<T>::type (&xv)[NV],
                                                 typename Vec16<T>::type (&acc)[NV], double (&sacc)[NSX], T *s_part,
                                                 T *s_u, int &slot) {
  using V = typename Vec16<T>::type;
  constexpr int VEC = Vec16<T>::N;
  constexpr int NW = TPB / 64;
  const int t = threadIdx.x, lane = t & 63, wave = t >> 6;
  const int nblk = (row_end - row_begin + RP - 1) / RP;
  int first = static_cast<int>(blockIdx.x) - blk_base % static_cast<int>(gridDim.x);
  if (first < 0) first += gridDim.x;
  for (int blk = first; blk < nblk; blk += gridDim.x, slot ^= 1) {
    const int row0 = row_begin + blk * RP;
    V av[RP][NVP];
#pragma unroll
    for (int r = 0; r < RP; ++r) {
      const int row = row0 + r;
      const T *rp = a.A + static_cast<size_t>(row) * a.lda;
#pragma unroll
      for (int v = 0; v < NVP; ++v) {
        const int col = (v * TPB + t) * VEC;
        V val = dev::vzero<V>();
        if (row < row_end && col <= row) val = *reinterpret_cast<const V *>(rp + col);
        av[r][v] = val;
      }
    }
    T p[RP];
#pragma unroll
    for (int r = 0; r < RP; ++r) {
      T s = 0;
#pragma unroll
      for (int v = 0; v < NVP; ++v) s += dev::vdot(av[r][v], xv[v]);
      p[r] = dev::wave_sum(s);
    }
    if (lane == 0) {
#pragma unroll
      for (int r = 0; r < RP; ++r) s_part[(slot * RMAX + r) * NW + wave] = p[r];
    }
    __syncthreads();
    if (t < RP) {
      const int row = row0 + t;
      T uval = 0;
      if (row < row_end) {
        T dot = 0;
#pragma unroll
        for (int w = 0; w < NW; ++w) dot += s_part[(slot * RMAX + t) * NW + w];
        uval = op.row(row, dot, sacc);
      }
      s_u[slot * RMAX + t] = uval;
    }
    __syncthreads();
#pragma unroll
    for (int r = 0; r < RP; ++r) {
      const T u = s_u[slot * RMAX + r];
#pragma unroll
      for (int v = 0; v < NVP; ++v) dev::vfma(acc[v], u, av[r][v]);
    }
  }
}

template <int NV> struct TriPhases {
  static constexpr int q = NV / 4;
  static constexpr int h = (NV / 2 > q) ? NV / 2 : 0;
};
template <int TPB, int NV, int VEC, int R>
__host__ __device__ inline void tri_phase_bounds(int m, int (&row)[4], int (&base)[3]) {
  constexpr int q = TriPhases<NV>::q, h = TriPhases<NV>::h;
  row[0] = 0;
  row[1] = q > 0 ? (q * TPB * VEC < m ? q * TPB * VEC : m) : 0;
  row[2] = h > 0 ? (h * TPB * VEC < m ? h * TPB * VEC : m) : row[1];
  row[3] = m;
  base[0] = 0;
  base[1] = (row[1] - row[0] + 4 * R - 1) / (4 * R);
  base[2] = base[1] + (row[2] - row[1] + 2 * R - 1) / (2 * R);
}

template <typename T, int TPB, int NV, int R, typename Op>
__global__ void __launch_bounds__(TPB) stream_tri_kernel(StreamArgs<T> a, Op op) {
  using V = typename Vec16<T>::type;
  constexpr int VEC = Vec16<T>::N;
  constexpr int NW = TPB / 64;
  constexpr int NS = Op::NS > 0 ? Op::NS : 1;
  constexpr int NVQ = TriPhases<NV>::q, NVH = TriPhases<NV>::h;
  constexpr int RMAX = NVQ > 0 ? 4 * R : (NVH > 0 ? 2 * R : R);
  __shared__ T s_part[2 * RMAX * NW];
  __shared__ T s_u[2 * RMAX];
  __shared__ double s_red[NS * NW];
  const int t = threadIdx.x;

  V xv[NV];
  V acc[NV];
  T sc = 1;
  if (a.xin_nrm2) sc = static_cast<T>(1.0 / sqrt(*a.xin_nrm2));
#pragma unroll
  for (int v = 0; v < NV; ++v) {
    const int col = (v * TPB + t) * VEC;
    V x = dev::vzero<V>();
    if (col < a.n_pad) {
      x = *reinterpret_cast<const V *>(a.xin + col);
      V add = dev::vzero<V>();
      if (a.xin_add) add = *reinterpret_cast<const V *>(a.xin_add + col);
      x = dev::vscale_add(x, sc, add);
    }
    xv[v] = x;
    acc[v] = dev::vzero<V>();
  }
  double sacc[NS];
#pragma unroll
  for (int k = 0; k < NS; ++k) sacc[k] = 0.0;

  int row[4], base[3];
  tri_phase_bounds<TPB, NV, VEC, R>(a.m, row, base);
  int slot = 0;
  if constexpr (NVQ > 0)
    stream_tri_phase<T, TPB, NV, 4 * R, NVQ, RMAX>(a, op, row[0], row[1], base[0], xv, acc, sacc, s_part, s_u, slot);
  if constexpr (NVH > 0)
    stream_tri_phase<T, TPB, NV, 2 * R, NVH, RMAX>(a, op, row[1], row[2], base[1], xv, acc, sacc, s_part, s_u, slot);
  stream_tri_phase<T, TPB, NV, R, NV, RMAX>(a, op, row[2], row[3], base[2], xv, acc, sacc, s_part, s_u, slot);

  T *out = a.col_partials + static_cast<size_t>(blockIdx.x) * a.n_pad;
#pragma unroll
  for (int v = 0; v < NV; ++v) {
    const int col = (v * TPB + t) * VEC;
    if (col < a.n_pad) *reinterpret_cast<V *>(out + col) = acc[v];
  }
  if (Op::NS > 0) {
    __syncthreads();
    dev::block_sum<NS, TPB>(sacc, s_red);
    if (t == 0) {
#pragma unroll
      for (int k = 0; k < NS; ++k) a.scalar_partials[static_cast<size_t>(blockIdx.x) * NS + k] = sacc[k];
    }
  }
}
template <bool DOT, bool ACC, int TPB>
struct RowsPerStep {
  static constexpr int value = (TPB == 1024) ? ((DOT && ACC) ? 1 : 2) : ((DOT && ACC) ? 2 : 4);
};

template <bool DOT, bool ACC>
inline int stream_grid(const StreamPlan &p, int m) {
  const int R = (p.tpb == 1024) ? ((DOT && ACC) ? 1 : 2) : ((DOT && ACC) ? 2 : 4);
  const int nblk = (m + R - 1) / R;
  return nblk < p.grid_dot ? (nblk > 0 ? nblk : 1) : p.grid_dot;
}

template <typename T>
struct XlStoreDotOp {
  static constexpr int NS = 0;
  T *out;
  template <int N>
  __device__ __forceinline__ T row(int i, T dot, double (&)[N]) const {
    out[i] = dot;
    return 0;
  }
  __device__ __forceinline__ T u(int) const { return 0; }
};
template <typename T>
struct XlVecUOp {
  static constexpr int NS = 0;
  const T *uvec;
  template <int N>
  __device__ __forceinline__ T row(int, T, double (&)[N]) const { return 0; }
  __device__ __forceinline__ T u(int i) const { return uvec[i]; }
};
template <typename T, typename Op, bool KEEP_U>
__global__ void __launch_bounds__(256) xl_apply_rows_kernel(const T *part, int m, int nwin, Op op, T *uvec,
                                                            double *scalar_partials) {
  constexpr int NS = Op::NS > 0 ? Op::NS : 1;
  __shared__ double s_red[NS * 4];
  double sacc[NS];
#pragma unroll
  for (int k = 0; k < NS; ++k) sacc[k] = 0.0;
  for (int i = blockIdx.x * 256 + threadIdx.x; i < m; i += gridDim.x * 256) {
    T dot = part[i];
    for (int c = 1; c < nwin; ++c) dot += part[static_cast<size_t>(c) * m + i];
    const T u = op.row(i, dot, sacc);
    if (KEEP_U) uvec[i] = u;
  }
  if (Op::NS > 0) {
    dev::block_sum<NS, 256>(sacc, s_red);
    if (threadIdx.x == 0) {
#pragma unroll
      for (int k = 0; k < NS; ++k) scalar_partials[static_cast<size_t>(blockIdx.x) * NS + k] = sacc[k];
    }
  }
}

template <typename T, bool DOT, bool ACC, bool SQ, int TRI, typename Tag, typename Op>
void launch_stream_plain(const StreamPlan &p, const StreamArgs<T> &a, const Op &op, hipStream_t s, int grid) {
#define POGS_STREAM_CASE(TPB_, NV_)                                                             \
  if constexpr (Tag::has(TPB_, NV_)) {                                                          \
    if (p.tpb == TPB_ && p.nv == NV_) {                                                         \
      constexpr int R_ = RowsPerStep<DOT, ACC, TPB_>::value;                                    \
       \
      if constexpr (DOT && ACC && !SQ && TRI == kLower && !(TPB_ == 1024 && NV_ == 8)) {        \
        if (a.col0 == 0) {                                              \
          hipLaunchKernelGGL((stream_tri_kernel<T, TPB_, NV_, R_, Op>), dim3(grid), dim3(TPB_), 0, s, a, op); \
          return;                                                                               \
        }                                                                                       \
      }                                                                                         \
      hipLaunchKernelGGL((stream_rows_kernel<T, TPB_, NV_, R_, DOT, ACC, SQ, TRI, Op>),         \
                         dim3(grid), dim3(TPB_), 0, s, a, op);                                  \
      return;                                                                                   \
    }                                                                                           \
  }
  POGS_STREAM_PLANS(POGS_STREAM_CASE)
#undef POGS_STREAM_CASE
  throw Error("no stream kernel instance for this plan in this translation unit");
}

template <typename T, bool DOT, bool ACC, bool SQ, int TRI, typename Tag, typename Op>
void launch_stream_window(const StreamPlan &p, const StreamArgs<T> &a, const Op &op, hipStream_t s, int grid) {
  if constexpr (Tag::windows) {
    if (p.tpb == 256 && p.nv == 8) {
      hipLaunchKernelGGL((stream_rows_kernel<T, 256, 8, RowsPerStep<DOT, ACC, 256>::value, DOT, ACC, SQ, TRI, Op>),
                         dim3(grid), dim3(256), 0, s, a, op);
      return;
    }
    if (p.tpb == 64 && p.nv == 2) {
      hipLaunchKernelGGL((stream_rows_kernel<T, 64, 2, RowsPerStep<DOT, ACC, 64>::value, DOT, ACC, SQ, TRI, Op>),
                         dim3(grid), dim3(64), 0, s, a, op);
      return;
    }
  }
  throw Error("no window kernel instance for this plan in this translation unit");
}

template <typename T, bool DOT, bool ACC, bool SQ, int TRI, typename Tag = AllPlans, typename Op>
void launch_stream(const StreamPlan &p, const StreamArgs<T> &a, const Op &op, hipStream_t s) {
  POGS_CHECK(p.ok, "matrix too wide for the row-streaming kernel");
  const int grid = stream_grid<DOT, ACC>(p, a.m);
  if (!p.xl) {
    launch_stream_plain<T, DOT, ACC, SQ, TRI, Tag, Op>(p, a, op, s, grid);
    return;
  }
  POGS_CHECK(a.xl_scratch != nullptr, "windowed pass without scratch");
  const int w = stream_window_cols<T>(p);
  const int nwin = stream_windows<T>(p, a.n_pad);
  T *part = a.xl_scratch, *uvec = a.xl_scratch + static_cast<size_t>(nwin) * a.m;
  StreamArgs<T> aw = a;
  if (DOT) {
    const int gdot = stream_grid<true, false>(p, a.m);
    for (int c = 0; c < nwin; ++c) {
      aw.col0 = c * w;
      launch_stream_window<T, true, false, SQ, TRI, Tag, XlStoreDotOp<T>>(p, aw, XlStoreDotOp<T>{part + static_cast<size_t>(c) * a.m},
                                                                     s, gdot);
    }
    hipLaunchKernelGGL((xl_apply_rows_kernel<T, Op, ACC>), dim3(grid), dim3(256), 0, s, part, a.m, nwin, op, uvec,
                       a.scalar_partials);
  }
  if (ACC) {
    for (int c = 0; c < nwin; ++c) {
      aw.col0 = c * w;
      if (DOT) launch_stream_window<T, false, true, SQ, TRI, Tag, XlVecUOp<T>>(p, aw, XlVecUOp<T>{uvec}, s, grid);
      else launch_stream_window<T, false, true, SQ, TRI, Tag, Op>(p, aw, op, s, grid);
    }
  }
}

template <typename T>
struct StreamArgs2 {
  const T *A;
  size_t lda;
  int m, n_pad;
  const T *xin0, *xin1;
  T *col_partials0, *col_partials1;
  double *scalar_partials;
};

template <typename T, int TPB, int NV, int R, int ND, int NA, typename Op>
__global__ void __launch_bounds__(TPB, (ND > 0 ? stream2_waves_per_simd(TPB, NV, ND, NA) : 1)) stream_rows2_kernel(StreamArgs2<T> a, Op op) {
  using V = typename Vec16<T>::type;
  constexpr int VEC = Vec16<T>::N;
  constexpr int NW = TPB / 64;
  constexpr int NS = Op::NS > 0 ? Op::NS : 1;
  constexpr int NDD = ND > 0 ? ND : 1;
  __shared__ T s_part[2 * R * NDD * NW];
  __shared__ T s_u[2 * R * NA];
  __shared__ double s_red[NS * NW];
  extern __shared__ __attribute__((aligned(16))) unsigned char s_dyn[];
  T *s_x1 = reinterpret_cast<T *>(s_dyn);
  const int t = threadIdx.x, lane = t & 63, wave = t >> 6;

  V xv[NV];
  V acc[NA][NV];
  if (ND > 0) {
#pragma unroll
    for (int v = 0; v < NV; ++v) {
      const int col = (v * TPB + t) * VEC;
      xv[v] = (col < a.n_pad) ? *reinterpret_cast<const V *>(a.xin0 + col) : dev::vzero<V>();
      if (ND > 1 && col < a.n_pad) *reinterpret_cast<V *>(s_x1 + col) = *reinterpret_cast<const V *>(a.xin1 + col);
    }
    if (ND > 1) __syncthreads();
  }
#pragma unroll
  for (int q = 0; q < NA; ++q)
#pragma unroll
    for (int v = 0; v < NV; ++v) acc[q][v] = dev::vzero<V>();
  double sacc[NS];
#pragma unroll
  for (int k = 0; k < NS; ++k) sacc[k] = 0.0;

  const int nblk = (a.m + R - 1) / R;
  int slot = 0;
  for (int blk = blockIdx.x; blk < nblk; blk += gridDim.x, slot ^= 1) {
    const int row0 = blk * R;
    V av[R][NV];
#pragma unroll
    for (int r = 0; r < R; ++r) {
      const int row = row0 + r;
      const T *rp = a.A + static_cast<size_t>(row) * a.lda;
#pragma unroll
      for (int v = 0; v < NV; ++v) {
        const int col = (v * TPB + t) * VEC;
        V val = dev::vzero<V>();
        if (col < a.n_pad && row < a.m) val = stream_load<V>(rp + col);
        av[r][v] = val;
      }
    }
    typename Op::Pre pre;
    if (ND > 0 && t < R && row0 + t < a.m) pre = op.prefetch(row0 + t);
    if (ND > 0) {
#pragma unroll
      for (int r = 0; r < R; ++r) {
        T s0 = 0, s1 = 0;
#pragma unroll
        for (int v = 0; v < NV; ++v) {
          s0 += dev::vdot(av[r][v], xv[v]);
          if (ND > 1) {
            const int col = (v * TPB + t) * VEC;
            if (col < a.n_pad) s1 += dev::vdot(av[r][v], *reinterpret_cast<const V *>(s_x1 + col));
          }
        }
        s0 = dev::wave_sum(s0);
        if (ND > 1) s1 = dev::wave_sum(s1);
        if (lane == 0) {
          s_part[((slot * R + r) * NDD + 0) * NW + wave] = s0;
          if (ND > 1) s_part[((slot * R + r) * NDD + 1) * NW + wave] = s1;
        }
      }
      __syncthreads();
      if (t < R) {
        const int row = row0 + t;
        T uu[NA];
#pragma unroll
        for (int q = 0; q < NA; ++q) uu[q] = 0;
        if (row < a.m) {
          T dots[NDD];
#pragma unroll
          for (int d = 0; d < ND; ++d) {
            T s = 0;
#pragma unroll
            for (int w = 0; w < NW; ++w) s += s_part[((slot * R + t) * NDD + d) * NW + w];
            dots[d] = s;
          }
          op.row(row, pre, dots, sacc, uu);
        }
#pragma unroll
        for (int q = 0; q < NA; ++q) s_u[(slot * R + t) * NA + q] = uu[q];
      }
      __syncthreads();
    }
#pragma unroll
    for (int r = 0; r < R; ++r) {
      T uu[NA];
      if (ND > 0) {
#pragma unroll
        for (int q = 0; q < NA; ++q) uu[q] = s_u[(slot * R + r) * NA + q];
      } else {
#pragma unroll
        for (int q = 0; q < NA; ++q) uu[q] = 0;
        if (row0 + r < a.m) op.uonly(row0 + r, uu);
      }
#pragma unroll
      for (int q = 0; q < NA; ++q)
#pragma unroll
        for (int v = 0; v < NV; ++v) dev::vfma(acc[q][v], uu[q], av[r][v]);
    }
  }
#pragma unroll
  for (int q = 0; q < NA; ++q) {
    T *out = (q == 0 ? a.col_partials0 : a.col_partials1) + static_cast<size_t>(blockIdx.x) * a.n_pad;
#pragma unroll
    for (int v = 0; v < NV; ++v) {
      const int col = (v * TPB + t) * VEC;
      if (col < a.n_pad) *reinterpret_cast<V *>(out + col) = acc[q][v];
    }
  }
  if (Op::NS > 0) {
    __syncthreads();
    dev::block_sum<NS, TPB>(sacc, s_red);
    if (t == 0) {
#pragma unroll
      for (int k = 0; k < NS; ++k) a.scalar_partials[static_cast<size_t>(blockIdx.x) * NS + k] = sacc[k];
    }
  }
}

#ifndef POGS_NV5_PREFETCH
#define POGS_NV5_PREFETCH 1
#endif
template <typename T, int TPB, int NV, int R, typename Op>
__global__ void __launch_bounds__(TPB, (2 * (TPB / 64) + 3) / 4) stream_rows2_pf_kernel(StreamArgs2<T> a, Op op) {
  using V = typename Vec16<T>::type;
  using Pre = typename Op::Pre;
  constexpr int VEC = Vec16<T>::N;
  constexpr int NW = TPB / 64;
  constexpr int NS = Op::NS > 0 ? Op::NS : 1;
  constexpr int ND = 2, NA = 2;
  __shared__ T s_part[2 * R * ND * NW];
  __shared__ T s_u[2 * R * NA];
  __shared__ double s_red[NS * NW];
  const int t = threadIdx.x, lane = t & 63, wave = t >> 6;

  V xv[NV], x1v[NV];
  V acc[NA][NV];
  int colc[NV];
#pragma unroll
  for (int v = 0; v < NV; ++v) {
    const int col = (v * TPB + t) * VEC;
    const bool in = col < a.n_pad;
    colc[v] = in ? col : a.n_pad - VEC;
    xv[v] = in ? *reinterpret_cast<const V *>(a.xin0 + col) : dev::vzero<V>();
    x1v[v] = in ? *reinterpret_cast<const V *>(a.xin1 + col) : dev::vzero<V>();
  }
#pragma unroll
  for (int q = 0; q < NA; ++q)
#pragma unroll
    for (int v = 0; v < NV; ++v) acc[q][v] = dev::vzero<V>();
  double sacc[NS];
#pragma unroll
  for (int k = 0; k < NS; ++k) sacc[k] = 0.0;

  const int nblk = (a.m + R - 1) / R;
  int blk = blockIdx.x;
  V cur[R][NV];
  Pre pre_cur;
  if (t < R && blk < nblk && blk * R + t < a.m) pre_cur = op.prefetch(blk * R + t);
#pragma unroll
  for (int r = 0; r < R; ++r) {
    const int row = blk * R + r;
    const T *rp = a.A + static_cast<size_t>(row < a.m ? row : a.m - 1) * a.lda;
#pragma unroll
    for (int v = 0; v < NV; ++v) cur[r][v] = stream_load<V>(rp + colc[v]);
  }
  int slot = 0;
  for (; blk < nblk; blk += gridDim.x, slot ^= 1) {
    const int row0 = blk * R;
    const int nblk_ = blk + gridDim.x, nrow0 = nblk_ * R;
    Pre pre_nxt;
    if (t < R && nblk_ < nblk && nrow0 + t < a.m) pre_nxt = op.prefetch(nrow0 + t);
    V nxt[R][NV];
#pragma unroll
    for (int r = 0; r < R; ++r) {
      const int row = nrow0 + r;
      const T *rp = a.A + static_cast<size_t>(row < a.m ? row : a.m - 1) * a.lda;
#pragma unroll
      for (int v = 0; v < NV; ++v) nxt[r][v] = stream_load<V>(rp + colc[v]);
    }
#pragma unroll
    for (int r = 0; r < R; ++r) {
      T s0 = 0, s1 = 0;
#pragma unroll
      for (int v = 0; v < NV; ++v) {
        s0 += dev::vdot(cur[r][v], xv[v]);
        s1 += dev::vdot(cur[r][v], x1v[v]);
      }
      s0 = dev::wave_sum_valu(s0);
      s1 = dev::wave_sum_valu(s1);
      if (lane == 0) {
        s_part[((slot * R + r) * ND + 0) * NW + wave] = s0;
        s_part[((slot * R + r) * ND + 1) * NW + wave] = s1;
      }
    }
    __syncthreads();
    if (t < R) {
      const int row = row0 + t;
      T uu[NA];
#pragma unroll
      for (int q = 0; q < NA; ++q) uu[q] = 0;
      if (row < a.m) {
        T dots[ND];
#pragma unroll
        for (int d = 0; d < ND; ++d) {
          T s = 0;
#pragma unroll
          for (int w = 0; w < NW; ++w) s += s_part[((slot * R + t) * ND + d) * NW + w];
          dots[d] = s;
        }
        op.row(row, pre_cur, dots, sacc, uu);
      }
#pragma unroll
      for (int q = 0; q < NA; ++q) s_u[(slot * R + t) * NA + q] = uu[q];
    }
    __syncthreads();
#pragma unroll
    for (int r = 0; r < R; ++r) {
      T uu[NA];
#pragma unroll
      for (int q = 0; q < NA; ++q) uu[q] = s_u[(slot * R + r) * NA + q];
#pragma unroll
      for (int q = 0; q < NA; ++q)
#pragma unroll
        for (int v = 0; v < NV; ++v) dev::vfma(acc[q][v], uu[q], cur[r][v]);
    }
#pragma unroll
    for (int r = 0; r < R; ++r)
#pragma unroll
      for (int v = 0; v < NV; ++v) cur[r][v] = nxt[r][v];
    pre_cur = pre_nxt;
  }
#pragma unroll
  for (int q = 0; q < NA; ++q) {
    T *out = (q == 0 ? a.col_partials0 : a.col_partials1) + static_cast<size_t>(blockIdx.x) * a.n_pad;
#pragma unroll
    for (int v = 0; v < NV; ++v) {
      const int col = (v * TPB + t) * VEC;
      if (col < a.n_pad) *reinterpret_cast<V *>(out + col) = acc[q][v];
    }
  }
  if (Op::NS > 0) {
    __syncthreads();
    dev::block_sum<NS, TPB>(sacc, s_red);
    if (t == 0) {
#pragma unroll
      for (int k = 0; k < NS; ++k) a.scalar_partials[static_cast<size_t>(blockIdx.x) * NS + k] = sacc[k];
    }
  }
}

inline bool stream2_supported(const StreamPlan &p) {
  if (!p.ok || p.xl) return false;
  if (p.tpb == 1024) return false;
  return p.nv <= 10;
}
constexpr int stream2_rows_c(int nd, int nv, int na = 2) {
  return nd > 0 ? ((nd == 1 && na == 1 && nv > 8) ? 2 : (nv <= 2 ? 8 : nv <= 4 ? 4 : nv == 5 ? 2 : nv <= 6 ? 3 : nv <= 8 ? 2 : 1))
                : (nv <= 4 ? 8 : nv <= 8 ? 4 : 2);
}
template <int ND, int NA = 2>
inline int stream2_rows(const StreamPlan &p) { return stream2_rows_c(ND, p.nv, NA); }
template <int ND, int NA = 2>
inline int stream2_grid(const StreamPlan &p, int m) {
  const int R = stream2_rows<ND, NA>(p);
  const int nblk = (m + R - 1) / R;
  const int gmax = ND > 0 ? (p.tpb == 256 && p.num_cu > 0
                                 ? p.num_cu * ((p.pf && ND == 2 && NA == 2) ? 2
                                               : p.bpc_override > 0         ? p.bpc_override
                                                                            : stream2_blocks_per_cu(256, p.nv, ND, NA))
                                 : p.grid_max)
                          : p.grid_dot;
  return nblk < gmax ? (nblk > 0 ? nblk : 1) : gmax;
}

template <typename T, int ND, int NA, typename Tag = AllPlans, typename Op>
void launch_stream2(const StreamPlan &p, const StreamArgs2<T> &a, const Op &op, hipStream_t s) {
  POGS_CHECK(stream2_supported(p), "plan not supported by the two-accumulator kernel");
  const int grid = stream2_grid<ND, NA>(p, a.m);
  if constexpr (ND == 2 && NA == 2 && std::is_same<T, float>::value && Tag::has(256, 5)) {
    if (p.pf && p.tpb == 256 && p.nv == 5) {
      hipLaunchKernelGGL((stream_rows2_pf_kernel<T, 256, 5, stream2_rows_c(2, 5, 2), Op>), dim3(grid), dim3(256), 0, s, a, op);
      return;
    }
  }
#define POGS_STREAM2_CASE(TPB_, NV_)                                                            \
  if constexpr (Tag::has(TPB_, NV_) && TPB_ != 1024)                                            \
  if (p.tpb == TPB_ && p.nv == NV_) {                                                           \
    constexpr int R_ = stream2_rows_c(ND, NV_, NA);                                             \
    const size_t lds = (ND > 1) ? static_cast<size_t>(a.n_pad) * sizeof(T) : 0;                 \
    static SmemGrants grants;                      \
    ensure_dynamic_smem(reinterpret_cast<const void *>(&stream_rows2_kernel<T, TPB_, NV_, R_, ND, NA, Op>), lds, grants); \
    hipLaunchKernelGGL((stream_rows2_kernel<T, TPB_, NV_, R_, ND, NA, Op>), dim3(grid),         \
                       dim3(TPB_), lds, s, a, op);                                              \
    return;                                                                                     \
  }
  POGS_STREAM_PLANS(POGS_STREAM2_CASE)
#undef POGS_STREAM2_CASE
  throw Error("no stream2 kernel instance for this plan in this translation unit");
}

template <typename T, typename ColOp>
__global__ void __launch_bounds__(256) reduce_cols_kernel(const T *partials, int nparts, int n_pad,
                                                          ColOp op, double *scalar_partials) {
  using V = typename Vec16<T>::type;
  constexpr int VEC = Vec16<T>::N;
  constexpr int NS = ColOp::NS > 0 ? ColOp::NS : 1;
  __shared__ V s_v[8][32];
  __shared__ double s_red[NS * 4];
  const int cx = threadIdx.x & 31, g = threadIdx.x >> 5;
  const int col = (blockIdx.x * 32 + cx) * VEC;
  V sum = dev::vzero<V>();
  if (col < n_pad) {
    int b = g;
    for (; b + 56 < nparts; b += 64) {
      V v[8];
#pragma unroll
      for (int q = 0; q < 8; ++q)
        v[q] = *reinterpret_cast<const V *>(partials + static_cast<size_t>(b + 8 * q) * n_pad + col);
#pragma unroll
      for (int q = 0; q < 8; ++q) dev::vadd(sum, v[q]);
    }
    for (; b < nparts; b += 8) {
      const V v = *reinterpret_cast<const V *>(partials + static_cast<size_t>(b) * n_pad + col);
      dev::vadd(sum, v);
    }
  }
  s_v[g][cx] = sum;
  __syncthreads();
  double sacc[NS];
#pragma unroll
  for (int k = 0; k < NS; ++k) sacc[k] = 0.0;
  if (g == 0 && col < n_pad) {
    V tot = s_v[0][cx];
#pragma unroll
    for (int q = 1; q < 8; ++q) dev::vadd(tot, s_v[q][cx]);
    const T *tp = reinterpret_cast<const T *>(&tot);
#pragma unroll
    for (int i = 0; i < VEC; ++i) op.col(col + i, tp[i], sacc);
  }
  if (ColOp::NS > 0) {
    __syncthreads();
    dev::block_sum<NS, 256>(sacc, s_red);
    if (threadIdx.x == 0) {
#pragma unroll
      for (int k = 0; k < NS; ++k) scalar_partials[static_cast<size_t>(blockIdx.x) * NS + k] = sacc[k];
    }
  }
}

inline int reduce_cols_grid(int n_pad, int vec) { return (n_pad / vec + 31) / 32; }

template <typename T, typename ColOp>
void launch_reduce_cols(const T *partials, int nparts, int n_pad, const ColOp &op,
                        double *scalar_partials, hipStream_t s) {
  const int grid = reduce_cols_grid(n_pad, Vec16<T>::N);
  hipLaunchKernelGGL((reduce_cols_kernel<T, ColOp>), dim3(grid), dim3(256), 0, s, partials, nparts,
                     n_pad, op, scalar_partials);
}

}
```

Baseline: 1538.

## Deepen column-partial reductions and batch triangular sweep x loads with check entrypoints

Column-partial reductions now issue batches of 32 (or 16) independent vector loads before accumulating, using two accumulators in the pre-cols path, so more memory requests are in flight per thread. The triangular streaming kernel loads x and its additive term unconditionally, clamping the index and masking afterwards, which removes branches around the loads. New check entrypoints compare the new and old variants for correctness. The cost is more registers per thread, which can reduce occupancy, and timing stamp hooks are added inside the kernel.

```diff
diff --git a/include/pogs_amd.h b/include/pogs_amd.h
--- a/include/pogs_amd.h
+++ b/include/pogs_amd.h
@@ -201,6 +201,11 @@
                void *y);
 int PogsAmdReadBandwidth(int device, size_t bytes, int reps, double *gb_per_s, int *pattern);
 int PogsAmdWaveSumCheck(int dtype, size_t n, const void *in_host, void *alu_host, void *lds_host);
+
+int PogsAmdTriSweepCheck(int dtype, int n, const void *M, size_t ldm, const void *x, int num_cu, void *out_new,
+                         void *out_old, void *dots_new, void *dots_old);
+int PogsAmdColSumCheck(int dtype, int nparts, int n_pad, const void *part0, const void *part1, void *tot_new,
+                       void *tot_old);
 
 int PogsAmdBatchRowsCheck(int dtype, int tri, int rows, int cols, const void *M, size_t ldm, int k, const int *act,
                           int nact, const void *X, size_t ldx, void *Y, size_t ldy);
diff --git a/pogs_amd/_lib.py b/pogs_amd/_lib.py
--- a/pogs_amd/_lib.py
+++ b/pogs_amd/_lib.py
@@ -135,6 +135,8 @@
 lib.PogsAmdRandUniform.argtypes = [c_int, c_size_t, c_void_p]
 lib.PogsAmdReadBandwidth.argtypes = [c_int, c_size_t, c_int, ctypes.POINTER(c_double), ctypes.POINTER(c_int)]
 lib.PogsAmdWaveSumCheck.argtypes = [c_int, c_size_t, c_void_p, c_void_p, c_void_p]
+lib.PogsAmdTriSweepCheck.argtypes = [c_int, c_int, c_void_p, c_size_t, c_void_p, c_int, c_void_p, c_void_p, c_void_p, c_void_p]
+lib.PogsAmdColSumCheck.argtypes = [c_int, c_int, c_int, c_void_p, c_void_p, c_void_p, c_void_p]
 lib.PogsAmdBatchRowsCheck.argtypes = [c_int, c_int, c_int, c_int, c_void_p, c_size_t, c_int, c_void_p, c_int,
                                       c_void_p, c_size_t, c_void_p, c_size_t]
 lib.PogsAmdBatchColsCheck.argtypes = [c_int, c_int, c_int, c_void_p, c_size_t, c_int, c_void_p, c_int, c_void_p,
@@ -189,7 +191,7 @@
     "PogsAmdIterate", "PogsAmdSetWarmStart", "PogsAmdGetStats", "PogsAmdResetStats", "PogsAmdDestroy", "PogsAmdLastError",
     "PogsAmdPoolStats", "PogsAmdPoolTrim",
     "PogsAmdProxEval", "PogsAmdFuncEval", "PogsAmdProjSubgradEval", "PogsAmdGetEquil", "PogsAmdProject", "PogsAmdMul", "PogsAmdRandUniform",
-    "PogsAmdReadBandwidth", "PogsAmdWaveSumCheck", "PogsAmdBatchRowsCheck", "PogsAmdBatchColsCheck",
+    "PogsAmdReadBandwidth", "PogsAmdWaveSumCheck", "PogsAmdTriSweepCheck", "PogsAmdColSumCheck", "PogsAmdBatchRowsCheck", "PogsAmdBatchColsCheck",
     "PogsAmdSpBatchSpmvCheck", "PogsAmdManySetupCheck", "PogsAmdGramCheck", "PogsAmdCholCheck",
     "PogsAmdSpmvCheck", "PogsAmdGetFactor",
 ]
@@ -210,6 +212,33 @@
     if lib.PogsAmdWaveSumCheck(0 if v.dtype == np.float32 else 1, v.size, v.ctypes.data, a.ctypes.data, b.ctypes.data) != 0:
         raise RuntimeError(last_error())
     return a, b
+
+
+def tri_sweep_check(M, x, num_cu=0):
+    import numpy as np
+    M, x = np.ascontiguousarray(M), np.ascontiguousarray(x)
+    code = _dtype_code(M, x)
+    if M.ndim != 2 or M.shape[0] != M.shape[1] or x.shape != (M.shape[0],):
+        raise ValueError("M (n, n), x (n,)")
+    outs = [np.empty(M.shape[0], dtype=M.dtype) for _ in range(4)]
+    if lib.PogsAmdTriSweepCheck(code, M.shape[0], M.ctypes.data, M.shape[1], x.ctypes.data, num_cu,
+                                *[o.ctypes.data for o in outs]) != 0:
+        raise RuntimeError(last_error())
+    return tuple(outs)
+
+
+def col_sum_check(part0, part1=None):
+    import numpy as np
+    part0 = np.ascontiguousarray(part0)
+    arrays = (part0,) if part1 is None else (part0, np.ascontiguousarray(part1))
+    code = _dtype_code(*arrays)
+    if part0.ndim != 2 or (part1 is not None and arrays[1].shape != part0.shape):
+        raise ValueError("part0 and part1 (nparts, n_pad)")
+    new, old = np.empty((4, part0.shape[1]), dtype=part0.dtype), np.empty((4, part0.shape[1]), dtype=part0.dtype)
+    if lib.PogsAmdColSumCheck(code, part0.shape[0], part0.shape[1], part0.ctypes.data,
+                              None if part1 is None else arrays[1].ctypes.data, new.ctypes.data, old.ctypes.data) != 0:
+        raise RuntimeError(last_error())
+    return new, old
 
 
 def _dtype_code(*arrays):
diff --git a/pogs_amd/csrc/abi.hip b/pogs_amd/csrc/abi.hip
--- a/pogs_amd/csrc/abi.hip
+++ b/pogs_amd/csrc/abi.hip
@@ -4,6 +4,7 @@
 #include <utility>
 #include <vector>
 
+#include "colside_check.h"
 #include "engine.h"
 #include "factor_check.h"
 #include "many_kernels.h"
@@ -22,6 +23,13 @@
                                                     const PogsAmdDist *);
 POGS_STREAM_PLANS(POGS_DECLARE_PLAN)
 #undef POGS_DECLARE_PLAN
+#define POGS_DECLARE_TRI_CHECK(TPB_, NV_)                                                                          \
+  void tri_sweep_check_f32_p##TPB_##_##NV_(const StreamPlan &, int, const void *, size_t, const void *, void *, void *, \
+                                           void *, void *);                                                        \
+  void tri_sweep_check_f64_p##TPB_##_##NV_(const StreamPlan &, int, const void *, size_t, const void *, void *, void *, \
+                                           void *, void *);
+POGS_STREAM_PLANS(POGS_DECLARE_TRI_CHECK)
+#undef POGS_DECLARE_TRI_CHECK
 SolverBase *make_dense_solver_f32_xl(int, size_t, size_t, const void *, int, const PogsAmdOptions *, const PogsAmdDist *);
 SolverBase *make_dense_solver_f64_xl(int, size_t, size_t, const void *, int, const PogsAmdOptions *, const PogsAmdDist *);
 
@@ -563,6 +571,50 @@
   });
 }
 
+int PogsAmdTriSweepCheck(int dtype, int n, const void *M, size_t ldm, const void *x, int num_cu, void *out_new,
+                         void *out_old, void *dots_new, void *dots_old) {
+  return guarded([&]() {
+    POGS_CHECK(dtype == POGS_AMD_F32 || dtype == POGS_AMD_F64, "unknown dtype");
+    POGS_CHECK(n >= 1 && num_cu >= 0, "n must be >= 1, num_cu >= 0");
+    POGS_CHECK(M && x && out_new && out_old && dots_new && dots_old, "null argument");
+    POGS_CHECK(ldm >= static_cast<size_t>(n), "ldm must be >= n");
+    if (num_cu == 0) {
+      int dev = 0;
+      hipDeviceProp_t prop;
+      POGS_HIP_CHECK(hipGetDevice(&dev));
+      POGS_HIP_CHECK(hipGetDeviceProperties(&prop, dev));
+      num_cu = prop.multiProcessorCount > 0 ? prop.multiProcessorCount : 256;
+    }
+    const bool f32 = dtype == POGS_AMD_F32;
+    const StreamPlan p = f32 ? make_stream_plan<float>(static_cast<int>(round_up(static_cast<size_t>(n), Vec16<float>::N)), num_cu)
+                             : make_stream_plan<double>(static_cast<int>(round_up(static_cast<size_t>(n), Vec16<double>::N)), num_cu);
+    POGS_CHECK(p.ok && !p.xl, "rows of n entries take the windowed form, which has no triangular sweep kernel");
+#define POGS_PICK_TRI_CHECK(TPB_, NV_)                                                                      \
+    if (p.tpb == TPB_ && p.nv == NV_) {                                                                     \
+      if (f32) tri_sweep_check_f32_p##TPB_##_##NV_(p, n, M, ldm, x, out_new, out_old, dots_new, dots_old);  \
+      else tri_sweep_check_f64_p##TPB_##_##NV_(p, n, M, ldm, x, out_new, out_old, dots_new, dots_old);      \
+      return 0;                                                                                             \
+    }
+    POGS_STREAM_PLANS(POGS_PICK_TRI_CHECK)
+#undef POGS_PICK_TRI_CHECK
+    throw Error("no triangular sweep for this streaming shape");
+  });
+}
+
+int PogsAmdColSumCheck(int dtype, int nparts, int n_pad, const void *part0, const void *part1, void *tot_new,
+                       void *tot_old) {
+  return guarded([&]() {
+    POGS_CHECK(dtype == POGS_AMD_F32 || dtype == POGS_AMD_F64, "unknown dtype");
+    if (dtype == POGS_AMD_F32)
+      col_sum_check<float>(nparts, n_pad, static_cast<const float *>(part0), static_cast<const float *>(part1),
+                           static_cast<float *>(tot_new), static_cast<float *>(tot_old));
+    else
+      col_sum_check<double>(nparts, n_pad, static_cast<const double *>(part0), static_cast<const double *>(part1),
+                            static_cast<double *>(tot_new), static_cast<double *>(tot_old));
+    return 0;
+  });
+}
+
 int PogsAmdBatchRowsCheck(int dtype, int tri, int rows, int cols, const void *M, size_t ldm, int k, const int *act,
                           int nact, const void *X, size_t ldx, void *Y, size_t ldy) {
   return guarded([&]() {
diff --git a/pogs_amd/csrc/colside_check.h b/pogs_amd/csrc/colside_check.h
--- /dev/null
+++ b/pogs_amd/csrc/colside_check.h
@@ -0,0 +1,111 @@
+#pragma once
+#include <vector>
+
+#include "common.h"
+#include "fused_cols.h"
+#include "stream.h"
+
+namespace pogs_amd {
+
+template <typename T>
+struct CheckStoreColOp {
+  static constexpr int NS = 0;
+  T *out;
+  template <int N>
+  __device__ __forceinline__ void col(int j, T total, double (&)[N]) const { out[j] = total; }
+};
+template <typename T>
+struct CheckDotRowOp {
+  static constexpr int NS = 0;
+  T *dots;
+  template <int N>
+  __device__ __forceinline__ T row(int i, T dot, double (&)[N]) const {
+    dots[i] = dot;
+    return dot;
+  }
+  __device__ __forceinline__ T u(int) const { return 0; }
+};
+
+template <typename T, bool DEEP>
+__global__ void __launch_bounds__(256) pre_cols_sums_kernel(const T *part0, const T *part1, int nparts, int n_pad,
+                                                            T *tot0, T *tot1) {
+  constexpr int NC = kPreColsVecs * Vec16<T>::N;
+  __shared__ __attribute__((aligned(16))) T s_v[2][kPreColsGroups][NC];
+  const int col0 = blockIdx.x * NC;
+  pre_cols_stage<T, DEEP, NC>(part0, part1, nparts, n_pad, col0, s_v);
+  const int j = col0 + static_cast<int>(threadIdx.x);
+  if (threadIdx.x < NC && j < n_pad) {
+    T t0, t1;
+    pre_cols_totals<T, NC>(s_v, t0, t1);
+    tot0[j] = t0;
+    tot1[j] = t1;
+  }
+}
+
+template <typename T>
+void col_sum_check(int nparts, int n_pad, const T *part0, const T *part1, T *tot_new, T *tot_old) {
+  constexpr int VEC = Vec16<T>::N;
+  POGS_CHECK(nparts >= 1 && n_pad >= VEC && n_pad % VEC == 0, "nparts must be >= 1, n_pad a positive multiple of VEC");
+  POGS_CHECK(part0 && tot_new && tot_old, "null argument");
+  const size_t np = static_cast<size_t>(nparts) * n_pad, nt = static_cast<size_t>(4) * n_pad;
+  DevBuf<T> d0(np), d1(part1 ? np : 0), tn(nt), to(nt);
+  hipStream_t s = nullptr;
+  POGS_HIP_CHECK(hipMemcpy(d0.p, part0, np * sizeof(T), hipMemcpyHostToDevice));
+  if (part1) POGS_HIP_CHECK(hipMemcpy(d1.p, part1, np * sizeof(T), hipMemcpyHostToDevice));
+  tn.zero(s);
+  to.zero(s);
+  const int grid = pre_cols_grid(n_pad, VEC);
+  launch_reduce_cols<T, CheckStoreColOp<T>, true>(d0.p, nparts, n_pad, CheckStoreColOp<T>{tn.p}, nullptr, s);
+  launch_reduce_cols<T, CheckStoreColOp<T>, false>(d0.p, nparts, n_pad, CheckStoreColOp<T>{to.p}, nullptr, s);
+  if (part1) {
+    launch_reduce_cols<T, CheckStoreColOp<T>, true>(d1.p, nparts, n_pad, CheckStoreColOp<T>{tn.p + n_pad}, nullptr, s);
+    launch_reduce_cols<T, CheckStoreColOp<T>, false>(d1.p, nparts, n_pad, CheckStoreColOp<T>{to.p + n_pad}, nullptr, s);
+  }
+  hipLaunchKernelGGL((pre_cols_sums_kernel<T, true>), dim3(grid), dim3(256), 0, s, d0.p, part1 ? d1.p : nullptr, nparts,
+                     n_pad, tn.p + 2 * static_cast<size_t>(n_pad), tn.p + 3 * static_cast<size_t>(n_pad));
+  hipLaunchKernelGGL((pre_cols_sums_kernel<T, false>), dim3(grid), dim3(256), 0, s, d0.p, part1 ? d1.p : nullptr, nparts,
+                     n_pad, to.p + 2 * static_cast<size_t>(n_pad), to.p + 3 * static_cast<size_t>(n_pad));
+  POGS_HIP_CHECK(hipGetLastError());
+  POGS_HIP_CHECK(hipMemcpy(tot_new, tn.p, nt * sizeof(T), hipMemcpyDeviceToHost));
+  POGS_HIP_CHECK(hipMemcpy(tot_old, to.p, nt * sizeof(T), hipMemcpyDeviceToHost));
+  POGS_HIP_CHECK(hipDeviceSynchronize());
+}
+
+template <typename T, typename Tag>
+void tri_sweep_check_t(const StreamPlan &p, int n, const T *M, size_t ldm, const T *x, T *out_new, T *out_old,
+                       T *dots_new, T *dots_old) {
+  constexpr size_t VEC = Vec16<T>::N;
+  const size_t ld = round_up(static_cast<size_t>(n), VEC);
+  std::vector<T> slab(static_cast<size_t>(n) * ld, static_cast<T>(0)), xp(ld, static_cast<T>(0));
+  for (int r = 0; r < n; ++r) {
+    const size_t vend = (static_cast<size_t>(r) / VEC + 1) * VEC;
+    for (size_t c = 0; c < static_cast<size_t>(n); ++c)
+      if (c <= static_cast<size_t>(r) || c >= vend) slab[r * ld + c] = M[r * ldm + c];
+  }
+  for (int c = 0; c < n; ++c) xp[c] = x[c];
+  const int grid = stream_grid<true, true>(p, n);
+  DevBuf<T> dM(slab.size()), dx(ld), part(static_cast<size_t>(grid) * ld), res(2 * (ld + n));
+  hipStream_t s = nullptr;
+  POGS_HIP_CHECK(hipMemcpy(dM.p, slab.data(), slab.size() * sizeof(T), hipMemcpyHostToDevice));
+  POGS_HIP_CHECK(hipMemcpy(dx.p, xp.data(), ld * sizeof(T), hipMemcpyHostToDevice));
+  res.zero(s);
+  T *o_new = res.p, *o_old = res.p + ld, *d_new = res.p + 2 * ld, *d_old = d_new + n;
+  StreamArgs<T> a;
+  a.A = dM.p; a.lda = ld; a.m = n; a.n_pad = static_cast<int>(ld);
+  a.xin = dx.p; a.xin_add = nullptr; a.xin_nrm2 = nullptr;
+  a.col_partials = part.p; a.scalar_partials = nullptr;
+  part.zero(s);
+  launch_stream<T, true, true, false, kLower, Tag, true>(p, a, CheckDotRowOp<T>{d_new}, s);
+  launch_reduce_cols<T, CheckStoreColOp<T>, true>(part.p, grid, a.n_pad, CheckStoreColOp<T>{o_new}, nullptr, s);
+  part.zero(s);
+  launch_stream<T, true, true, false, kLower, Tag, false>(p, a, CheckDotRowOp<T>{d_old}, s);
+  launch_reduce_cols<T, CheckStoreColOp<T>, false>(part.p, grid, a.n_pad, CheckStoreColOp<T>{o_old}, nullptr, s);
+  POGS_HIP_CHECK(hipGetLastError());
+  POGS_HIP_CHECK(hipMemcpy(out_new, o_new, n * sizeof(T), hipMemcpyDeviceToHost));
+  POGS_HIP_CHECK(hipMemcpy(out_old, o_old, n * sizeof(T), hipMemcpyDeviceToHost));
+  POGS_HIP_CHECK(hipMemcpy(dots_new, d_new, n * sizeof(T), hipMemcpyDeviceToHost));
+  POGS_HIP_CHECK(hipMemcpy(dots_old, d_old, n * sizeof(T), hipMemcpyDeviceToHost));
+  POGS_HIP_CHECK(hipDeviceSynchronize());
+}
+
+}
diff --git a/pogs_amd/csrc/dense_plan.hip b/pogs_amd/csrc/dense_plan.hip
--- a/pogs_amd/csrc/dense_plan.hip
+++ b/pogs_amd/csrc/dense_plan.hip
@@ -1,3 +1,4 @@
+#include "colside_check.h"
 #include "dense_solver.h"
 
 #define POGS_CAT2(a, b) a##b
@@ -13,4 +14,12 @@
                                                           const PogsAmdOptions *opt, const PogsAmdDist *dist) {
   return make_dense_solver_t<POGS_PLAN_T, PlanTag>(ord, m, n, A, mem, opt, dist);
 }
+#if !defined(POGS_PLAN_XL)
+void POGS_CAT(tri_sweep_check_, POGS_PLAN_NAME)(const StreamPlan &p, int n, const void *M, size_t ldm, const void *x,
+                                                void *out_new, void *out_old, void *dots_new, void *dots_old) {
+  using T = POGS_PLAN_T;
+  tri_sweep_check_t<T, PlanTag>(p, n, static_cast<const T *>(M), ldm, static_cast<const T *>(x), static_cast<T *>(out_new),
+                                static_cast<T *>(out_old), static_cast<T *>(dots_new), static_cast<T *>(dots_old));
 }
+#endif
+}
diff --git a/pogs_amd/csrc/fused_cols.h b/pogs_amd/csrc/fused_cols.h
--- a/pogs_amd/csrc/fused_cols.h
+++ b/pogs_amd/csrc/fused_cols.h
@@ -8,25 +8,6 @@
 #include "vec_kernels.h"
 
 namespace pogs_amd {
-
-template <typename T>
-__device__ __forceinline__ typename Vec16<T>::type colsum_group(const T *partials, int nparts, int n_pad, int col, int g) {
-  using V = typename Vec16<T>::type;
-  V sum = dev::vzero<V>();
-  int b = g;
-  for (; b + 56 < nparts; b += 64) {
-    V v[8];
-#pragma unroll
-    for (int q = 0; q < 8; ++q) v[q] = *reinterpret_cast<const V *>(partials + static_cast<size_t>(b + 8 * q) * n_pad + col);
-#pragma unroll
-    for (int q = 0; q < 8; ++q) dev::vadd(sum, v[q]);
-  }
-  for (; b < nparts; b += 8) {
-    const V v = *reinterpret_cast<const V *>(partials + static_cast<size_t>(b) * n_pad + col);
-    dev::vadd(sum, v);
-  }
-  return sum;
-}
 
 template <typename T>
 struct PreColsArgs {
@@ -45,53 +26,77 @@
 constexpr int kPreColsVecs = 16, kPreColsGroups = 16;
 inline int pre_cols_grid(int n_pad, int vec) { return (n_pad / vec + kPreColsVecs - 1) / kPreColsVecs; }
 
-template <typename T, bool SRC64>
+template <typename T, int NB>
+__device__ __forceinline__ void pre_colsum_batch(const T *part, int n_pad, int col, int b, typename Vec16<T>::type &s,
+                                                 typename Vec16<T>::type &t) {
+  using V = typename Vec16<T>::type;
+  V v[NB];
+#pragma unroll
+  for (int q = 0; q < NB; ++q) v[q] = *reinterpret_cast<const V *>(part + static_cast<size_t>(b + q * kPreColsGroups) * n_pad + col);
+  dev::requests_before(s);
+  dev::requests_before(t);
+#pragma unroll
+  for (int q = 0; q < NB; q += 2) {
+    dev::vadd(s, v[q]);
+    dev::vadd(t, v[q + 1]);
+  }
+}
+template <typename T, bool DEEP>
+__device__ __forceinline__ typename Vec16<T>::type pre_colsum_group(const T *part, int nparts, int n_pad, int col, int g) {
+  using V = typename Vec16<T>::type;
+  constexpr int G = kPreColsGroups;
+  V s = dev::vzero<V>(), t = dev::vzero<V>();
+  int b = g;
+  if constexpr (DEEP) {
+    for (; b + 31 * G < nparts; b += 32 * G) pre_colsum_batch<T, 32>(part, n_pad, col, b, s, t);
+    for (; b + 15 * G < nparts; b += 16 * G) pre_colsum_batch<T, 16>(part, n_pad, col, b, s, t);
+  }
+  for (; b + G < nparts; b += 2 * G) {
+    const V u = *reinterpret_cast<const V *>(part + static_cast<size_t>(b) * n_pad + col);
+    const V w = *reinterpret_cast<const V *>(part + static_cast<size_t>(b + G) * n_pad + col);
+    dev::vadd(s, u);
+    dev::vadd(t, w);
+  }
+  if (b < nparts) dev::vadd(s, *reinterpret_cast<const V *>(part + static_cast<size_t>(b) * n_pad + col));
+  dev::vadd(s, t);
+  return s;
+}
+
+template <typename T, bool DEEP, int NC>
+__device__ __forceinline__ void pre_cols_stage(const T *part0, const T *part1, int nparts, int n_pad, int col0,
+                                               T (&s_v)[2][kPreColsGroups][NC]) {
+  using V = typename Vec16<T>::type;
+  constexpr int VEC = Vec16<T>::N;
+  const int cx = threadIdx.x % kPreColsVecs, g = threadIdx.x / kPreColsVecs;
+  const int col = col0 + cx * VEC;
+  V s0 = dev::vzero<V>(), s1 = dev::vzero<V>();
+  if (col < n_pad) {
+    s0 = pre_colsum_group<T, DEEP>(part0, nparts, n_pad, col, g);
+    if (part1) s1 = pre_colsum_group<T, DEEP>(part1, nparts, n_pad, col, g);
+  }
+  *reinterpret_cast<V *>(&s_v[0][g][cx * VEC]) = s0;
+  *reinterpret_cast<V *>(&s_v[1][g][cx * VEC]) = s1;
+  __syncthreads();
+}
+template <typename T, int NC>
+__device__ __forceinline__ void pre_cols_totals(const T (&s_v)[2][kPreColsGroups][NC], T &t0, T &t1) {
+  t0 = s_v[0][0][threadIdx.x];
+  t1 = s_v[1][0][threadIdx.x];
+#pragma unroll
+  for (int q = 1; q < kPreColsGroups; ++q) {
+    t0 += s_v[0][q][threadIdx.x];
+    t1 += s_v[1][q][threadIdx.x];
+  }
+}
+
+template <typename T, bool SRC64, bool DEEP = true>
 __global__ void __launch_bounds__(256) pre_cols_kernel(PreColsArgs<T> a) {
-  using V = typename Vec16<T>::type;
   constexpr int VEC = Vec16<T>::N;
   constexpr int NC = kPreColsVecs * VEC;
-  __shared__ T s_v[2][kPreColsGroups][NC];
+  __shared__ __attribute__((aligned(16))) T s_v[2][kPreColsGroups][NC];
   __shared__ double s_red[4 * 4];
-  const int cx = threadIdx.x % kPreColsVecs, g = threadIdx.x / kPreColsVecs;
   const int col0 = blockIdx.x * NC;
-  if (!SRC64) {
-    const int col = col0 + cx * VEC;
-    V s0 = dev::vzero<V>(), s1 = dev::vzero<V>();
-    if (col < a.n_pad) {
-      V t0 = dev::vzero<V>(), t1 = dev::vzero<V>();
-      int b = g;
-      if (a.part1) {
-        for (; b + kPreColsGroups < a.nparts; b += 2 * kPreColsGroups) {
-          const V u0 = *reinterpret_cast<const V *>(a.part0 + static_cast<size_t>(b) * a.n_pad + col);
-          const V u1 = *reinterpret_cast<const V *>(a.part1 + static_cast<size_t>(b) * a.n_pad + col);
-          const V w0 = *reinterpret_cast<const V *>(a.part0 + static_cast<size_t>(b + kPreColsGroups) * a.n_pad + col);
-          const V w1 = *reinterpret_cast<const V *>(a.part1 + static_cast<size_t>(b + kPreColsGroups) * a.n_pad + col);
-          dev::vadd(s0, u0);
-          dev::vadd(s1, u1);
-          dev::vadd(t0, w0);
-          dev::vadd(t1, w1);
-        }
-        if (b < a.nparts) {
-          dev::vadd(s0, *reinterpret_cast<const V *>(a.part0 + static_cast<size_t>(b) * a.n_pad + col));
-          dev::vadd(s1, *reinterpret_cast<const V *>(a.part1 + static_cast<size_t>(b) * a.n_pad + col));
-        }
-      } else {
-        for (; b + kPreColsGroups < a.nparts; b += 2 * kPreColsGroups) {
-          const V u0 = *reinterpret_cast<const V *>(a.part0 + static_cast<size_t>(b) * a.n_pad + col);
-          const V w0 = *reinterpret_cast<const V *>(a.part0 + static_cast<size_t>(b + kPreColsGroups) * a.n_pad + col);
-          dev::vadd(s0, u0);
-          dev::vadd(t0, w0);
-        }
-        if (b < a.nparts)
-          dev::vadd(s0, *reinterpret_cast<const V *>(a.part0 + static_cast<size_t>(b) * a.n_pad + col));
-      }
-      dev::vadd(s0, t0);
-      dev::vadd(s1, t1);
-    }
-    *reinterpret_cast<V *>(&s_v[0][g][cx * VEC]) = s0;
-    *reinterpret_cast<V *>(&s_v[1][g][cx * VEC]) = s1;
-    __syncthreads();
-  }
+  if (!SRC64) pre_cols_stage<T, DEEP, NC>(a.part0, a.part1, a.nparts, a.n_pad, col0, s_v);
   double sacc[4] = {0.0, 0.0, 0.0, 0.0};
   const int j = col0 + static_cast<int>(threadIdx.x);
   if (threadIdx.x < NC && j < a.n_pad) {
@@ -100,13 +105,7 @@
       t0 = static_cast<T>(a.tot64[j]);
       t1 = static_cast<T>(a.tot64[a.n_pad + j]);
     } else {
-      t0 = s_v[0][0][threadIdx.x];
-      t1 = s_v[1][0][threadIdx.x];
-#pragma unroll
-      for (int q = 1; q < kPreColsGroups; ++q) {
-        t0 += s_v[0][q][threadIdx.x];
-        t1 += s_v[1][q][threadIdx.x];
-      }
+      pre_cols_totals<T, NC>(s_v, t0, t1);
     }
     if (j < a.n) {
       const T prev = a.x_cur[j];
diff --git a/pogs_amd/csrc/stream.h b/pogs_amd/csrc/stream.h
--- a/pogs_amd/csrc/stream.h
+++ b/pogs_amd/csrc/stream.h
@@ -161,6 +161,12 @@
 __device__ __forceinline__ double2 vscale_add(const double2 &a, double s, const double2 &b) {
   return make_double2(fma_(a.x, s, b.x), fma_(a.y, s, b.y));
 }
+__device__ __forceinline__ void requests_before(float4 &acc) {
+  asm volatile("" : "+v"(acc.x), "+v"(acc.y), "+v"(acc.z), "+v"(acc.w) : : "memory");
+}
+__device__ __forceinline__ void requests_before(double2 &acc) {
+  asm volatile("" : "+v"(acc.x), "+v"(acc.y) : : "memory");
+}
 template <typename V> __device__ __forceinline__ V vzero();
 template <> __device__ __forceinline__ float4 vzero<float4>() { return make_float4(0.f, 0.f, 0.f, 0.f); }
 template <> __device__ __forceinline__ double2 vzero<double2>() { return make_double2(0.0, 0.0); }
@@ -282,6 +288,21 @@
       for (int k = 0; k < NS; ++k) a.scalar_partials[static_cast<size_t>(blockIdx.x) * NS + k] = sacc[k];
     }
   }
+}
+
+#ifndef POGS_TRI_STAMP
+#define POGS_TRI_STAMP(k)
+#endif
+template <typename V>
+__device__ __forceinline__ V tri_keep(const V &v, bool keep) {
+  typedef unsigned int raw16 __attribute__((ext_vector_type(4)));
+  static_assert(sizeof(V) == 16, "16-byte vectors");
+  raw16 raw;
+  __builtin_memcpy(&raw, &v, 16);
+  raw &= keep ? ~0u : 0u;
+  V out;
+  __builtin_memcpy(&out, &raw, 16);
+  return out;
 }
 
 template <typename T, int TPB, int NV, int RP, int NVP, int RMAX, int NSX, typename Op>
@@ -311,6 +332,8 @@
         av[r][v] = val;
       }
     }
+    POGS_TRI_STAMP(2);
+    POGS_TRI_STAMP(3);
     T p[RP];
 #pragma unroll
     for (int r = 0; r < RP; ++r) {
@@ -323,7 +346,9 @@
 #pragma unroll
       for (int r = 0; r < RP; ++r) s_part[(slot * RMAX + r) * NW + wave] = p[r];
     }
+    POGS_TRI_STAMP(4);
     __syncthreads();
+    POGS_TRI_STAMP(5);
     if (t < RP) {
       const int row = row0 + t;
       T uval = 0;
@@ -335,13 +360,16 @@
       }
       s_u[slot * RMAX + t] = uval;
     }
+    POGS_TRI_STAMP(6);
     __syncthreads();
+    POGS_TRI_STAMP(7);
 #pragma unroll
     for (int r = 0; r < RP; ++r) {
       const T u = s_u[slot * RMAX + r];
 #pragma unroll
       for (int v = 0; v < NVP; ++v) dev::vfma(acc[v], u, av[r][v]);
     }
+    POGS_TRI_STAMP(8);
   }
 }
 
@@ -361,7 +389,7 @@
   base[2] = base[1] + (row[2] - row[1] + 2 * R - 1) / (2 * R);
 }
 
-template <typename T, int TPB, int NV, int R, typename Op>
+template <typename T, int TPB, int NV, int R, typename Op, bool XB = true>
 __global__ void __launch_bounds__(TPB) stream_tri_kernel(StreamArgs<T> a, Op op) {
   using V = typename Vec16<T>::type;
   constexpr int VEC = Vec16<T>::N;
@@ -373,24 +401,45 @@
   __shared__ T s_u[2 * RMAX];
   __shared__ double s_red[NS * NW];
   const int t = threadIdx.x;
+  POGS_TRI_STAMP(0);
 
   V xv[NV];
   V acc[NV];
   T sc = 1;
   if (a.xin_nrm2) sc = static_cast<T>(1.0 / sqrt(*a.xin_nrm2));
-#pragma unroll
-  for (int v = 0; v < NV; ++v) {
-    const int col = (v * TPB + t) * VEC;
-    V x = dev::vzero<V>();
-    if (col < a.n_pad) {
-      x = *reinterpret_cast<const V *>(a.xin + col);
-      V add = dev::vzero<V>();
-      if (a.xin_add) add = *reinterpret_cast<const V *>(a.xin_add + col);
-      x = dev::vscale_add(x, sc, add);
-    }
-    xv[v] = x;
-    acc[v] = dev::vzero<V>();
-  }
+  if constexpr (XB) {
+    const T *addp = a.xin_add ? a.xin_add : a.xin;
+    const bool has_add = a.xin_add != nullptr;
+    V xr[NV], ar[NV];
+#pragma unroll
+    for (int v = 0; v < NV; ++v) {
+      const int col = (v * TPB + t) * VEC;
+      const int cc = col < a.n_pad ? col : a.n_pad - VEC;
+      xr[v] = *reinterpret_cast<const V *>(a.xin + cc);
+      ar[v] = *reinterpret_cast<const V *>(addp + cc);
+    }
+#pragma unroll
+    for (int v = 0; v < NV; ++v) {
+      const int col = (v * TPB + t) * VEC;
+      xv[v] = tri_keep(dev::vscale_add(xr[v], sc, tri_keep(ar[v], has_add)), col < a.n_pad);
+      acc[v] = dev::vzero<V>();
+    }
+  } else {
+#pragma unroll
+    for (int v = 0; v < NV; ++v) {
+      const int col = (v * TPB + t) * VEC;
+      V x = dev::vzero<V>();
+      if (col < a.n_pad) {
+        x = *reinterpret_cast<const V *>(a.xin + col);
+        V add = dev::vzero<V>();
+        if (a.xin_add) add = *reinterpret_cast<const V *>(a.xin_add + col);
+        x = dev::vscale_add(x, sc, add);
+      }
+      xv[v] = x;
+      acc[v] = dev::vzero<V>();
+    }
+  }
+  POGS_TRI_STAMP(1);
   double sacc[NS];
 #pragma unroll
   for (int k = 0; k < NS; ++k) sacc[k] = 0.0;
@@ -404,12 +453,14 @@
     stream_tri_phase<T, TPB, NV, 2 * R, NVH, RMAX>(a, op, row[1], row[2], base[1], xv, acc, sacc, s_part, s_u, slot);
   stream_tri_phase<T, TPB, NV, R, NV, RMAX>(a, op, row[2], row[3], base[2], xv, acc, sacc, s_part, s_u, slot);
 
+  POGS_TRI_STAMP(9);
   T *out = a.col_partials + static_cast<size_t>(blockIdx.x) * a.n_pad;
 #pragma unroll
   for (int v = 0; v < NV; ++v) {
     const int col = (v * TPB + t) * VEC;
     if (col < a.n_pad) *reinterpret_cast<V *>(out + col) = acc[v];
   }
+  POGS_TRI_STAMP(10);
   if (Op::NS > 0) {
     __syncthreads();
     dev::block_sum<NS, TPB>(sacc, s_red);
@@ -473,7 +524,7 @@
   }
 }
 
-template <typename T, bool DOT, bool ACC, bool SQ, int TRI, typename Tag, typename Op>
+template <typename T, bool DOT, bool ACC, bool SQ, int TRI, typename Tag, typename Op, bool TRI_XB = true>
 void launch_stream_plain(const StreamPlan &p, const StreamArgs<T> &a, const Op &op, hipStream_t s, int grid) {
 #define POGS_STREAM_CASE(TPB_, NV_)                                                             \
   if constexpr (Tag::has(TPB_, NV_)) {                                                          \
@@ -482,7 +533,7 @@
        \
       if constexpr (DOT && ACC && !SQ && TRI == kLower && !(TPB_ == 1024 && NV_ == 8)) {        \
         if (a.col0 == 0) {                                              \
-          hipLaunchKernelGGL((stream_tri_kernel<T, TPB_, NV_, R_, Op>), dim3(grid), dim3(TPB_), 0, s, a, op); \
+          hipLaunchKernelGGL((stream_tri_kernel<T, TPB_, NV_, R_, Op, TRI_XB>), dim3(grid), dim3(TPB_), 0, s, a, op); \
           return;                                                                               \
         }                                                                                       \
       }                                                                                         \
@@ -513,12 +564,12 @@
   throw Error("no window kernel instance for this plan in this translation unit");
 }
 
-template <typename T, bool DOT, bool ACC, bool SQ, int TRI, typename Tag = AllPlans, typename Op>
+template <typename T, bool DOT, bool ACC, bool SQ, int TRI, typename Tag = AllPlans, bool TRI_XB = true, typename Op>
 void launch_stream(const StreamPlan &p, const StreamArgs<T> &a, const Op &op, hipStream_t s) {
   POGS_CHECK(p.ok, "matrix too wide for the row-streaming kernel");
   const int grid = stream_grid<DOT, ACC>(p, a.m);
   if (!p.xl) {
-    launch_stream_plain<T, DOT, ACC, SQ, TRI, Tag, Op>(p, a, op, s, grid);
+    launch_stream_plain<T, DOT, ACC, SQ, TRI, Tag, Op, TRI_XB>(p, a, op, s, grid);
     return;
   }
   POGS_CHECK(a.xl_scratch != nullptr, "windowed pass without scratch");
@@ -866,7 +917,36 @@
   throw Error("no stream2 kernel instance for this plan in this translation unit");
 }
 
-template <typename T, typename ColOp>
+template <typename T, bool DEEP = true>
+__device__ __forceinline__ typename Vec16<T>::type colsum_group(const T *partials, int nparts, int n_pad, int col, int g) {
+  using V = typename Vec16<T>::type;
+  V sum = dev::vzero<V>();
+  int b = g;
+  if constexpr (DEEP) {
+    for (; b + 8 * 31 < nparts; b += 8 * 32) {
+      V v[32];
+#pragma unroll
+      for (int q = 0; q < 32; ++q) v[q] = *reinterpret_cast<const V *>(partials + static_cast<size_t>(b + 8 * q) * n_pad + col);
+      dev::requests_before(sum);
+#pragma unroll
+      for (int q = 0; q < 32; ++q) dev::vadd(sum, v[q]);
+    }
+  }
+  for (; b + 56 < nparts; b += 64) {
+    V v[8];
+#pragma unroll
+    for (int q = 0; q < 8; ++q) v[q] = *reinterpret_cast<const V *>(partials + static_cast<size_t>(b + 8 * q) * n_pad + col);
+#pragma unroll
+    for (int q = 0; q < 8; ++q) dev::vadd(sum, v[q]);
+  }
+  for (; b < nparts; b += 8) {
+    const V v = *reinterpret_cast<const V *>(partials + static_cast<size_t>(b) * n_pad + col);
+    dev::vadd(sum, v);
+  }
+  return sum;
+}
+
+template <typename T, typename ColOp, bool DEEP = true>
 __global__ void __launch_bounds__(256) reduce_cols_kernel(const T *partials, int nparts, int n_pad,
                                                           ColOp op, double *scalar_partials) {
   using V = typename Vec16<T>::type;
@@ -877,21 +957,7 @@
   const int cx = threadIdx.x & 31, g = threadIdx.x >> 5;
   const int col = (blockIdx.x * 32 + cx) * VEC;
   V sum = dev::vzero<V>();
-  if (col < n_pad) {
-    int b = g;
-    for (; b + 56 < nparts; b += 64) {
-      V v[8];
-#pragma unroll
-      for (int q = 0; q < 8; ++q)
-        v[q] = *reinterpret_cast<const V *>(partials + static_cast<size_t>(b + 8 * q) * n_pad + col);
-#pragma unroll
-      for (int q = 0; q < 8; ++q) dev::vadd(sum, v[q]);
-    }
-    for (; b < nparts; b += 8) {
-      const V v = *reinterpret_cast<const V *>(partials + static_cast<size_t>(b) * n_pad + col);
-      dev::vadd(sum, v);
-    }
-  }
+  if (col < n_pad) sum = colsum_group<T, DEEP>(partials, nparts, n_pad, col, g);
   s_v[g][cx] = sum;
   __syncthreads();
   double sacc[NS];
@@ -917,11 +983,11 @@
 
 inline int reduce_cols_grid(int n_pad, int vec) { return (n_pad / vec + 31) / 32; }
 
-template <typename T, typename ColOp>
+template <typename T, typename ColOp, bool DEEP = true>
 void launch_reduce_cols(const T *partials, int nparts, int n_pad, const ColOp &op,
                         double *scalar_partials, hipStream_t s) {
   const int grid = reduce_cols_grid(n_pad, Vec16<T>::N);
-  hipLaunchKernelGGL((reduce_cols_kernel<T, ColOp>), dim3(grid), dim3(256), 0, s, partials, nparts,
+  hipLaunchKernelGGL((reduce_cols_kernel<T, ColOp, DEEP>), dim3(grid), dim3(256), 0, s, partials, nparts,
                      n_pad, op, scalar_partials);
 }
 
```

Result: slower. 1517 (-1.4%).
